# mfkiwl/HiSpMV

Measured on AMD Instinct MI355X. Metric: SpMV GFLOP/s, SuiteSparse set (20 matrices), fp32 y=alpha*A*x+beta*y, flops=2*(nnz+rows), higher is better.
Workload: dtype f32

## Files before the change

hispmv_amd/_lib.py:

```python
from __future__ import annotations

import ctypes as C
import os
from pathlib import Path

_HERE = Path(__file__).resolve().parent
LIB_PATH = Path(os.environ.get("HISPMV_LIB", _HERE / "lib" / "libhispmv.so"))

HISPMV_OK = 0
HISPMV_FULL = -1
HISPMV_EINVAL = -2
HISPMV_EDEVICE = -3
HISPMV_ESTATE = -4
HISPMV_ENOTDENSE = -5
HISPMV_EIO = -6
HISPMV_ENOMEM = -7


class MatrixInfo(C.Structure):
    _fields_ = [
        ("rows", C.c_int32), ("cols", C.c_int32), ("nnz", C.c_int64),
        ("is_dense", C.c_int32), ("loaded", C.c_int32),
        ("n_slices", C.c_int64), ("n_elems", C.c_int64), ("n_split_rows", C.c_int64),
        ("device_bytes", C.c_int64), ("prep_seconds", C.c_double),
        ("block_threads", C.c_int32), ("group_slices", C.c_int32), ("lds_bytes", C.c_int32), ("col_tiles", C.c_int32),
        ("carry_lookback", C.c_int32), ("col_tile_width", C.c_int32),
        ("col_tile_base", C.c_int32), ("compact_slices", C.c_int32),
        ("format", C.c_int32), ("tts_lines_per_gather", C.c_float), ("tile_kind", C.c_int32),
        ("batch_group_slices", C.c_int32),
    ]


_p = C.c_void_p
_i32p = C.POINTER(C.c_int32)
_i64p = C.POINTER(C.c_int64)
_u64p = C.POINTER(C.c_uint64)
_f32p = C.POINTER(C.c_float)

SIGNATURES = {
    "hispmv_prep_build_tts": (C.c_int, [_p, C.c_int64, C.c_int, C.POINTER(C.c_int64), C.POINTER(C.c_double)]),
    "hispmv_prep_tts_array": (C.c_void_p, [_p, C.c_int]),
    "hispmv_prep_tts_pieces": (C.c_int, [_p, C.POINTER(C.c_int64)]),
    "hispmv_version": (C.c_char_p, []),
    "hispmv_host_threads": (C.c_int, []),
    "hispmv_free_failures": (C.c_int64, []),
    "hispmv_boundary_pack": (C.c_int, [C.c_void_p, C.c_void_p, C.c_void_p, C.c_void_p, C.c_int32, C.c_void_p]),
    "hispmv_boundary_apply": (C.c_int, [C.c_void_p, C.c_void_p, C.c_void_p, C.c_void_p, C.c_int32, C.c_int32, C.c_void_p]),
    "hispmv_create": (C.c_int, [C.POINTER(_p), C.c_char_p] + [C.c_int] * 9),
    "hispmv_destroy": (None, [_p]),
    "hispmv_last_error": (C.c_char_p, [_p]),
    "hispmv_set_arena_bytes": (C.c_int, [_p, C.c_int64]),
    "hispmv_arena_bytes_used": (C.c_int64, [_p]),
    "hispmv_create_sparse_handle": (C.c_int, [_p, _p, _p, _p, C.c_int64, C.c_int32, C.c_int32]),
    "hispmv_create_sparse_handle_from_mtx": (C.c_int, [_p, C.c_char_p, C.c_int]),
    "hispmv_create_sparse_handle_from_csr": (C.c_int, [_p, _p, _p, _p, C.c_int32, C.c_int32]),
    "hispmv_create_dense_handle": (C.c_int, [_p, _p, C.c_int32, C.c_int32]),
    "hispmv_load_matrices": (C.c_int, [_p]),
    "hispmv_select_matrix": (C.c_int, [_p, C.c_uint32]),
    "hispmv_run_kernel": (C.c_int, [_p, _p, _p, _p, C.c_float, C.c_float]),
    "hispmv_linear": (C.c_int, [_p, C.c_int, _p, C.c_int64, _p, _p]),
    "hispmv_spmv_device": (C.c_int, [_p, C.c_int, _p, _p, _p, C.c_float, C.c_float, _p]),
    "hispmv_synchronize": (C.c_int, [_p]),
    "hispmv_last_kernel_ms": (C.c_float, [_p]),
    "hispmv_batch_graph_stats": (C.c_int, [_p, C.POINTER(C.c_int64)]),
    "hispmv_batch_call_info": (C.c_int, [_p, C.POINTER(C.c_int64)]),
    "hispmv_spmv_device_batch": (C.c_int, [_p, C.c_int32, _p, _p, _p, _p, C.c_float, C.c_float, _p]),
    "hispmv_set_value_updates": (C.c_int, [_p, C.c_int]),
    "hispmv_update_values": (C.c_int, [_p, C.c_int, _p, C.c_int64]),
    "hispmv_update_values_device": (C.c_int, [_p, C.c_int, _p, C.c_int64, _p]),
    "hispmv_value_update_info": (C.c_int, [_p, C.c_int, _i64p]),
    "hispmv_time_device": (C.c_float, [_p, C.c_int, _p, _p, _p, C.c_float, C.c_float, C.c_int]),
    "hispmv_get_matrix_info": (C.c_int, [_p, C.c_int, C.POINTER(MatrixInfo)]),
    "hispmv_num_matrices": (C.c_int, [_p]),
    "hispmv_prep_from_coo": (C.c_int, [C.POINTER(_p), _p, _p, _p, C.c_int64, C.c_int32, C.c_int32]),
    "hispmv_prep_from_coo_device": (C.c_int, [C.POINTER(_p), C.c_int, _p, _p, _p, C.c_int64, C.c_int32, C.c_int32, C.POINTER(C.c_double)]),
    "hispmv_prep_from_mtx": (C.c_int, [C.POINTER(_p), C.c_char_p, C.c_int]),
    "hispmv_prep_free": (None, [_p]),
    "hispmv_prep_last_error": (C.c_char_p, []),
    "hispmv_prep_dims": (C.c_int, [_p, _i64p]),
    "hispmv_prep_plan": (C.c_int, [_p, C.c_int, _i64p]),
    "hispmv_prep_choose_format": (C.c_int, [_p, C.c_int, _i64p]),
    "hispmv_prep_step_queue": (C.c_int, [_p, C.c_int32, _p, C.c_int32, C.c_int32, C.c_int32, _p, _p]),
    "hispmv_prep_window_membership": (C.c_int, [_p, C.c_int, C.c_void_p]),
    "hispmv_prep_apply_plan": (C.c_int, [_p, C.c_int, _i64p]),
    "hispmv_prep_groups": (_i32p, [_p]),
    "hispmv_prep_device_stream": (C.c_int, [_p, _i64p]),
    "hispmv_prep_device_array": (C.c_void_p, [_p, C.c_int]),
    "hispmv_prep_device_stream_on_device": (C.c_int, [_p, C.c_int, C.c_void_p, C.c_void_p]),
    "hispmv_prep_frags": (_i32p, [_p]),
    "hispmv_prep_value_layouts": (C.c_int, [C.POINTER(_p), _p, _p, _p, C.c_int64, C.c_int32, C.c_int32, C.c_int, _i64p]),
    "hispmv_prep_value_array": (C.c_void_p, [_p, C.c_int]),
    "hispmv_prep_csr_row_ptr": (_i64p, [_p]),
    "hispmv_prep_csr_col": (_i32p, [_p]),
    "hispmv_prep_csr_val": (_f32p, [_p]),
    "hispmv_prep_words": (_u64p, [_p]),
    "hispmv_prep_slice_hdr": (_i32p, [_p]),
    "hispmv_prep_fix": (_i32p, [_p]),
}


def _bind_single_hip_runtime() -> None:
    import importlib.util
    spec = importlib.util.find_spec("torch")
    if spec is None or not spec.origin:
        return
    cand = Path(spec.origin).parent / "lib" / "libamdhip64.so"
    if cand.exists():
        C.CDLL(str(cand), mode=C.RTLD_GLOBAL)


def _load() -> C.CDLL:
    if not LIB_PATH.exists():
        raise ImportError(
            f"{LIB_PATH} not found: the HIP library is not built. Run "
            "`python -c 'import __graft_entry__ as g; g.build()'` (or `make -C hispmv_amd/csrc`). "
            "There is no CPU fallback."
        )
    _bind_single_hip_runtime()
    lib = C.CDLL(str(LIB_PATH))
    for name, (res, args) in SIGNATURES.items():
        fn = getattr(lib, name)
        fn.restype = res
        fn.argtypes = args
    return lib


lib = _load()
```

hispmv_amd/csrc/hispmv_abi.cpp:

```cpp
#include "hispmv_ctx.h"

using namespace hispmv;

namespace {

thread_local std::string g_create_err;
thread_local std::string g_prep_err;

}

namespace hispmv {
int fail(hispmv_ctx* c, int code, const std::string& msg) {
    if (c) c->err = msg; else g_create_err = msg;
    return code;
}
int hip_fail(hispmv_ctx* c, hipError_t e, const char* what) {
    return fail(c, HISPMV_EDEVICE, std::string(what) + ": " + hipGetErrorString(e));
}
std::string& prep_error() { return g_prep_err; }
std::atomic<int64_t> g_free_failures{0};
int check_device_error(hispmv_ctx* c) {
    const int flag = *(volatile int*)c->h_err;
    if (flag) {
        *(volatile int*)c->h_err = 0;
// ... 437 lines not shown
            const int rc = check_updatable(c, nnz);
            if (rc != HISPMV_OK) return rc;
        }
        csr.col.assign(ci, ci + nnz);
        if (c->value_updates) { real.assign(va, va + nnz); const std::vector<float> pl = index_payloads(nnz); csr.val.assign(pl.begin(), pl.end()); }
        else csr.val.assign(va, va + nnz);
        for (int64_t k = 0; k < nnz; ++k) if (ci[k] < 0 || ci[k] >= cols) return fail(c, HISPMV_EINVAL, "CSR column outside matrix");
        sort_rows_by_column(csr);
        double t = std::chrono::duration<double>(std::chrono::steady_clock::now() - t0).count();
        return add_sparse(c, std::move(csr), t, nullptr, c->value_updates ? &real : nullptr);
    } catch (const std::bad_alloc&) { return fail(c, HISPMV_ENOMEM, "host out of memory");
    } catch (const std::exception& ex) { return fail(c, HISPMV_EINVAL, ex.what()); }
}

HISPMV_API int hispmv_create_dense_handle(hispmv_ctx* c, const float* vals, int32_t rows, int32_t cols) {
    if (!c) return HISPMV_EINVAL;
    std::lock_guard<std::mutex> g(c->mu);
    if (!c->dense_overlay)
        return fail(c, HISPMV_ENOTDENSE, "Hardware is not built with Dense Overlay, cannot support dense workload");
    if (rows <= 0 || cols <= 0 || !vals) return fail(c, HISPMV_EINVAL, "bad dense matrix arguments");
    try {
        auto t0 = std::chrono::steady_clock::now();
        auto m = std::make_unique<Matrix>();
        m->dense = true; m->rows = rows; m->cols = cols; m->nnz = (int64_t)rows * cols;
        m->device_bytes = m->nnz * 4;
        if (c->arena_used + m->device_bytes > c->arena_budget) return HISPMV_FULL;
        m->dense_host.assign(vals, vals + m->nnz);
        if (c->value_updates) { m->updatable = true; m->upd_n = m->nnz; m->upd_written = m->nnz; }
        m->prep_seconds = std::chrono::duration<double>(std::chrono::steady_clock::now() - t0).count();
        c->arena_used += m->device_bytes;
        m->index = (int)c->mats.size();
    c->mats.push_back(std::move(m));
        return (int)c->mats.size() - 1;
    } catch (const std::bad_alloc&) { return fail(c, HISPMV_ENOMEM, "host out of memory"); }
}

HISPMV_API int hispmv_load_matrices(hispmv_ctx* c) {
    if (!c) return HISPMV_EINVAL;
    std::lock_guard<std::mutex> g(c->mu);
    HIP_TRY(c, hipSetDevice(c->device));
    for (auto& mp : c->mats) {
        Matrix& m = *mp;
        if (m.loaded) continue;
        int rc;
        struct Scratch { std::vector<void*> v; void push_back(void* p) { v.push_back(p); } ~Scratch() { for (void* p : v) (void)hipFree(p); } } layout_scratch;
        std::vector<std::vector<int32_t>> tts_fix_rows;
        std::vector<std::vector<ValueChunk>> value_regions;
        std::vector<std::pair<int64_t, int64_t>> layout_bytes;
        if (m.updatable && !m.dense)
            for (const Matrix::Part& p : m.parts) {
                value_regions.push_back(value_chunks(p));
                layout_bytes.emplace_back(p.is_tts ? (int64_t)p.tts.words.size() : p.dstream.n_bytes, p.has_batch_layout ? p.batch_dstream.n_bytes : 0);
            }
        if (m.dense) {
            const float* d = nullptr;
            if ((rc = upload(c, m, m.dense_host.data(), m.dense_host.size(), &d)) != HISPMV_OK) return rc;
            m.d_dense = const_cast<float*>(d);
        } else if (m.format == 1) {
          for (Matrix::Part& p : m.parts) {
            TtsStream& ts = p.tts;
            tts_fix_rows.emplace_back();
            for (size_t k = 0; k + 3 < ts.fix.size(); k += 4) tts_fix_rows.back().push_back(ts.fix[k]);
            const uint8_t* dw = nullptr; const int32_t* dcb = nullptr; const uint16_t* dfl = nullptr; const int32_t* dci = nullptr;
            const TtsTile* dt = nullptr; const TtsBlock* db = nullptr;
            if ((rc = upload(c, m, ts.words.data(), ts.words.size(), &dw)) != HISPMV_OK) return rc;
            if ((rc = upload(c, m, ts.col_base.data(), ts.col_base.size(), &dcb)) != HISPMV_OK) return rc;
            if ((rc = upload(c, m, ts.flags.data(), ts.flags.size(), &dfl)) != HISPMV_OK) return rc;
            const uint16_t* dfh = nullptr;
            std::vector<uint32_t> planes;
            if (!ts.flags_hi.empty()) {
                planes.resize(ts.flags.size());
                for (size_t q = 0; q < planes.size(); ++q) planes[q] = (uint32_t)ts.flags[q] | ((uint32_t)ts.flags_hi[q] << 16);
                const uint32_t* dp = nullptr;
                if ((rc = upload(c, m, planes.data(), planes.size(), &dp)) != HISPMV_OK) return rc;
                HIP_TRY(c, hipStreamSynchronize(c->stream));
                dfh = (const uint16_t*)dp;
            }
            if ((rc = upload(c, m, ts.chunk_info.data(), ts.chunk_info.size(), &dci)) != HISPMV_OK) return rc;
            if ((rc = upload(c, m, ts.tiles.data(), ts.tiles.size(), &dt)) != HISPMV_OK) return rc;
            if ((rc = upload(c, m, ts.blocks.data(), ts.blocks.size(), &db)) != HISPMV_OK) return rc;
            TtsDeviceMatrix& d = p.tdev;
            d.words = dw; d.col_base = dcb; d.flags = dfl; d.flags_hi = dfh; d.chunk_info = (const int2*)dci; d.tiles = (const int4*)dt; d.blocks = (const int4*)db;
            d.n_tiles = (int32_t)ts.tiles.size(); d.rows = m.rows; d.cols = m.cols;
            if (!ts.fix.empty()) {
                const int32_t* dfix = nullptr;
                if ((rc = upload(c, m, ts.fix.data(), ts.fix.size(), &dfix)) != HISPMV_OK) return rc;
                void* carry = nullptr;
                HIP_TRY(c, hipMalloc(&carry, (size_t)std::max(ts.n_carry, 1) * kTtsMaxVectors * sizeof(float)));
                m.allocs.push_back(carry);
                HIP_TRY(c, hipMemsetAsync(carry, 0, (size_t)std::max(ts.n_carry, 1) * kTtsMaxVectors * sizeof(float), c->stream));
                d.n_carry = ts.n_carry;
                d.fix = (const int4*)dfix; d.n_fix = (int32_t)(ts.fix.size() / 4); d.carry = (float*)carry;
                p.dev.fix_short = d.fix; p.dev.n_fix_short = d.n_fix; p.dev.carry = d.carry; p.dev.n_fix_long = 0;
            }
            d.acc_floats = (ts.max_rows + 63) & ~63; d.threads = ts.geometry.threads;
            d.zero_fill = ts.geometry.zero_fill ? 1 : ts.geometry.gap_rows ? 2 : 0;
            d.staging_floats = ts.geometry.max_slots + 64;
            d.batch_stage_floats = ((ts.max_slots + kTtsChunk - 1) / kTtsChunk) * kTtsChunk + 64;
            d.xlds_floats = (m.cols <= kTtsXldsMax && std::getenv("HISPMV_TTS_XLDS")) ? ((m.cols + 63) & ~63) : 0;
            if (((size_t)d.acc_floats + (size_t)d.staging_floats + 64) * 4 > 160 * 1024 - 256) return fail(c, HISPMV_EINVAL, "internal: tile stream exceeds the LDS of a CU");
            HIP_TRY(c, hipStreamSynchronize(c->stream));
            p.tts = TtsStream{};
          }
        } else {
            for (auto& p : m.parts) {
                const uint8_t* dw = nullptr; const SliceHdr* dh = nullptr; const FixEntry *fs = nullptr, *fl = nullptr;
                const int32_t* dg = nullptr; const Frag* dfr = nullptr;
                const int64_t ns = p.st.n_slices;
                if ((rc = upload(c, m, p.dstream.groups.data(), p.dstream.groups.size(), &dg)) != HISPMV_OK) return rc;
                if ((rc = upload(c, m, p.plan.frags.data(), p.plan.frags.size(), &dfr)) != HISPMV_OK) return rc;
                const bool lay_out = p.dstream.bytes.empty() && p.dstream.n_bytes > 0;
                uint64_t* d_host_words = nullptr;
                if (!lay_out) {
                    if ((rc = upload(c, m, p.dstream.bytes.data(), p.dstream.bytes.size(), &dw)) != HISPMV_OK) return rc;
                } else {
                    if ((int64_t)p.st.words.size() != ns * kSliceElems) return fail(c, HISPMV_EINVAL, "internal: host words missing for the device layout");
                    void* blk = nullptr;
                    HIP_TRY(c, hipMalloc(&blk, (size_t)p.dstream.n_bytes));
                    m.allocs.push_back(blk);
                    dw = (const uint8_t*)blk;
                    HIP_TRY(c, hipMalloc((void**)&d_host_words, p.st.words.size() * sizeof(uint64_t)));
                    layout_scratch.push_back(d_host_words);
                    HIP_TRY(c, hipMemcpyAsync(d_host_words, p.st.words.data(), p.st.words.size() * sizeof(uint64_t), hipMemcpyHostToDevice, c->stream));
                }
                std::vector<SliceHdr>& hh = p.st.hdr;
                int max_rows = 1;
                for (int64_t sl = 0; sl < ns; ++sl) {
                    const int nr = (sl + 1 < ns ? hh[sl + 1].row_base : m.rows) - hh[sl].row_base;
                    hh[sl].x_base = nr;
                    hh[sl].x_span = (!p.plan.slice_spills.empty() && p.plan.slice_spills[(size_t)sl]) ? 1 : 0;
                    max_rows = std::max(max_rows, nr);
                }
                uint32_t* d_stray_cols = nullptr;
                if (!p.dstream.any_stray) {
                    if ((rc = upload(c, m, hh.data(), hh.size(), &dh)) != HISPMV_OK) return rc;
                } else if (lay_out) {
                    void* blk = nullptr;
                    const size_t hb = hh.size() * sizeof(SliceHdr), sb = (size_t)ns * kStraySlots * sizeof(uint32_t);
                    HIP_TRY(c, hipMalloc(&blk, hb + sb));
                    m.allocs.push_back(blk);
                    HIP_TRY(c, hipMemcpyAsync(blk, hh.data(), hb, hipMemcpyHostToDevice, c->stream));
                    HIP_TRY(c, hipMemsetAsync((char*)blk + hb, 0xff, sb, c->stream));
                    dh = (const SliceHdr*)blk;
                    d_stray_cols = (uint32_t*)((char*)blk + hb);
                } else {
                    void* blk = nullptr;
                    const size_t hb = hh.size() * sizeof(SliceHdr), sb = p.dstream.stray_cols.size() * sizeof(uint32_t);
                    HIP_TRY(c, hipMalloc(&blk, hb + sb));
                    m.allocs.push_back(blk);
                    HIP_TRY(c, hipMemcpyAsync(blk, hh.data(), hb, hipMemcpyHostToDevice, c->stream));
                    HIP_TRY(c, hipMemcpyAsync((char*)blk + hb, p.dstream.stray_cols.data(), sb, hipMemcpyHostToDevice, c->stream));
                    dh = (const SliceHdr*)blk;
                }
                if (lay_out) {
                    const int e = layout_on_device(d_host_words, ns, p.plan.group_slices, dg, p.plan.lds_floats, p.plan.block_threads / 64,
                                                   (uint8_t*)dw, d_stray_cols, c->stream);
                    if (e != 0) return hip_fail(c, (hipError_t)e, "layout_on_device");
                }
                if ((rc = upload(c, m, p.fix_short.data(), p.fix_short.size(), &fs)) != HISPMV_OK) return rc;
                if ((rc = upload(c, m, p.fix_long.data(), p.fix_long.size(), &fl)) != HISPMV_OK) return rc;
                void *carry = nullptr, *gran = nullptr, *ticket = nullptr;
                const size_t n1 = (size_t)std::max<int64_t>(ns, 1);
                HIP_TRY(c, hipMalloc(&carry, n1 * kMaxBatch * sizeof(float)));
                m.allocs.push_back(carry);
                HIP_TRY(c, hipMemsetAsync(carry, 0, n1 * kMaxBatch * sizeof(float), c->stream));
                HIP_TRY(c, hipMalloc(&gran, n1 * sizeof(unsigned long long)));
                m.allocs.push_back(gran);
                HIP_TRY(c, hipMemsetAsync(gran, 0, n1 * sizeof(unsigned long long), c->stream));
                HIP_TRY(c, hipMalloc(&ticket, sizeof(unsigned long long)));
                m.allocs.push_back(ticket);
                HIP_TRY(c, hipMemsetAsync(ticket, 0, sizeof(unsigned long long), c->stream));
                SpmvDeviceMatrix& d = p.dev;
                d.words = dw; d.hdr = (const int4*)dh; d.groups = (const int4*)dg; d.frags = (const int4*)dfr;
                d.fix_short = (const int4*)fs; d.fix_long = (const int4*)fl;
                d.carry = (float*)carry; d.gran = (unsigned long long*)gran; d.ticket = (unsigned long long*)ticket;
                d.err = c->d_err; d.launches = 0; d.ticket_launches = 0;
                d.n_slices = ns; d.n_groups = (ns + p.plan.group_slices - 1) / p.plan.group_slices;
                d.group_slices = p.plan.group_slices; d.block_threads = p.plan.block_threads;
                d.lds_floats = p.plan.lds_floats + p.dstream.stray_floats;
                d.ytile_floats = std::min(kSliceElems, (max_rows + 63) & ~63);
                const size_t lds_plain = (size_t)(d.lds_floats + d.ytile_floats * (d.block_threads / 64)) * 4;
                if (lds_plain > 160 * 1024 - 256) return fail(c, HISPMV_EINVAL, "internal: launch plan exceeds the LDS of a CU");
                const bool mailbox_fits = lds_plain + (size_t)d.group_slices * 8 <= 160 * 1024 - 256;
                d.n_fix_short = (int32_t)p.fix_short.size(); d.n_fix_long = (int32_t)p.fix_long.size();
                d.rows = m.rows; d.cols = m.cols;
                const int lds_b = std::max(1, (int)lds_plain + 64);
                const int per_cu = std::max(1, std::min({4, (160 * 1024) / lds_b, 16 / (d.block_threads / 64)}));
                const bool resident = d.n_groups <= (int64_t)c->n_cus * per_cu;
                const bool one_round = d.group_slices <= d.block_threads / 64;
                d.lookback = (c->carry_mode == 1 || c->carry_mode == 3 || (c->carry_mode == 2 && resident && one_round) ||
                              (c->carry_mode == 5 && resident)) && mailbox_fits;
                d.use_ticket = c->carry_mode == 3;
                if (m.parts.size() > 1) { d.lookback = false; d.use_ticket = false; }
                d.has_strays = p.dstream.stray_floats > 0;
                if (d.has_strays) { d.lookback = false; d.use_ticket = false; }
                if (p.has_batch_layout) {
                    SpmvDeviceMatrix b = d;
                    const int32_t* bg = nullptr; const Frag* bf = nullptr; const uint8_t* bw = nullptr; const SliceHdr* bh = nullptr;
                    if ((rc = upload(c, m, p.batch_dstream.groups.data(), p.batch_dstream.groups.size(), &bg)) != HISPMV_OK) return rc;
                    if ((rc = upload(c, m, p.batch_plan.frags.data(), p.batch_plan.frags.size(), &bf)) != HISPMV_OK) return rc;
                    std::vector<SliceHdr> bhh = hh;
                    for (int64_t sl = 0; sl < ns; ++sl) bhh[(size_t)sl].x_span = (!p.batch_plan.slice_spills.empty() && p.batch_plan.slice_spills[(size_t)sl]) ? 1 : 0;
                    uint32_t* b_stray = nullptr;
                    {
                        void* blk = nullptr;
                        const size_t hb = bhh.size() * sizeof(SliceHdr), sb = p.batch_dstream.any_stray ? (size_t)ns * kStraySlots * sizeof(uint32_t) : 0;
                        HIP_TRY(c, hipMalloc(&blk, hb + sb));
                        m.allocs.push_back(blk);
                        HIP_TRY(c, hipMemcpy(blk, bhh.data(), hb, hipMemcpyHostToDevice));
                        if (sb && !p.batch_dstream.stray_cols.empty()) HIP_TRY(c, hipMemcpy((char*)blk + hb, p.batch_dstream.stray_cols.data(), sb, hipMemcpyHostToDevice));
                        else if (sb) HIP_TRY(c, hipMemsetAsync((char*)blk + hb, 0xff, sb, c->stream));
                        bh = (const SliceHdr*)blk;
                        b_stray = sb ? (uint32_t*)((char*)blk + hb) : nullptr;
                    }
                    if (!p.batch_dstream.bytes.empty()) {
                        if ((rc = upload(c, m, p.batch_dstream.bytes.data(), p.batch_dstream.bytes.size(), &bw)) != HISPMV_OK) return rc;
                    } else {
                        void* blk = nullptr; uint64_t* tmp = nullptr;
                        HIP_TRY(c, hipMalloc(&blk, (size_t)p.batch_dstream.n_bytes));
                        m.allocs.push_back(blk);
                        bw = (const uint8_t*)blk;
                        HIP_TRY(c, hipMalloc((void**)&tmp, p.batch_words.size() * sizeof(uint64_t)));
                        layout_scratch.push_back(tmp);
                        HIP_TRY(c, hipMemcpyAsync(tmp, p.batch_words.data(), p.batch_words.size() * sizeof(uint64_t), hipMemcpyHostToDevice, c->stream));
                        const int e = layout_on_device(tmp, ns, p.batch_plan.group_slices, bg, p.batch_plan.lds_floats, p.batch_plan.block_threads / 64, (uint8_t*)blk, b_stray, c->stream);
                        if (e != 0) return hip_fail(c, (hipError_t)e, "layout_on_device");
                    }
                    b.words = bw; b.hdr = (const int4*)bh; b.groups = (const int4*)bg; b.frags = (const int4*)bf;
                    b.group_slices = p.batch_plan.group_slices; b.n_groups = (ns + p.batch_plan.group_slices - 1) / p.batch_plan.group_slices;
                    b.lds_floats = p.batch_plan.lds_floats + p.batch_dstream.stray_floats;
                    b.has_strays = p.batch_dstream.stray_floats > 0;
                    b.lookback = false; b.use_ticket = false;
                    if ((size_t)(b.lds_floats + b.ytile_floats * (b.block_threads / 64)) * 4 <= 160 * 1024 - 256) { p.batch_dev = b; p.has_batch_dev = true; }
                }
            }
        }
        if (!m.dense && m.parts.size() > 1) {
            void* yp = nullptr;
            HIP_TRY(c, hipMalloc(&yp, (m.parts.size() - 1) * (size_t)kMaxBatch * m.rows * sizeof(float)));
            m.allocs.push_back(yp);
            m.d_ypart = (float*)yp;
            bool fusable = m.parts.size() <= (size_t)kTailMaxParts;
            for (auto& p : m.parts) fusable = fusable && (p.is_tts || p.fix_long.empty());
            if (fusable) {
                std::vector<int32_t> of((size_t)m.parts.size() * m.rows, -1);
                for (size_t t = 0; t < m.parts.size(); ++t) {
                    int32_t* o = of.data() + t * (size_t)m.rows;
                    if (m.parts[t].is_tts) { const std::vector<int32_t>& f = tts_fix_rows[t]; for (size_t k = 0; k < f.size(); ++k) o[f[k]] = (int32_t)k; }
                    else for (size_t k = 0; k < m.parts[t].fix_short.size(); ++k) o[m.parts[t].fix_short[k].row] = (int32_t)k;
                }
                const int32_t* d_of = nullptr;
                if ((rc = upload(c, m, of.data(), of.size(), &d_of)) != HISPMV_OK) return rc;
                HIP_TRY(c, hipStreamSynchronize(c->stream));
                m.d_fix_of_row = const_cast<int32_t*>(d_of);
            }
        }
        if (m.updatable && !m.dense && (rc = load_value_map(c, m, value_regions, layout_bytes)) != HISPMV_OK) return rc;
        HIP_TRY(c, hipStreamSynchronize(c->stream));
        for (auto& p : m.parts) { p.st = SliceStream{}; p.fix_short = {}; p.fix_long = {}; p.plan.groups = {}; p.plan.frags = {}; p.dstream = DeviceStream{};
                                  p.batch_plan.groups = {}; p.batch_plan.frags = {}; p.batch_plan.slice_spills = {}; p.batch_dstream = DeviceStream{}; p.batch_words = WordVec(); }
        m.dense_host = {};
        m.loaded = true;
    }
    return HISPMV_OK;
}

HISPMV_API int hispmv_select_matrix(hispmv_ctx* c, uint32_t idx) {
    if (!c) return HISPMV_EINVAL;
    std::lock_guard<std::mutex> g(c->mu);
    if (idx >= c->mats.size()) return fail(c, HISPMV_EINVAL, "Matrix idx out of range");
    c->selected = (int)idx;
    return HISPMV_OK;
}

static int run_host_vectors(hispmv_ctx* c, Matrix& m, const float* x, int64_t num_vecs, const float* bias,
                            float* y, float alpha, float beta, bool is_linear) {
    HIP_TRY(c, hipSetDevice(c->device));
    int rc;
    const int64_t nx = (((int64_t)m.cols * num_vecs + 63) / 64) * 64, nb = m.rows, ny = (int64_t)m.rows * num_vecs;
    if ((rc = ensure_vec(c, &c->d_x, &c->cap_x, nx + nb)) != HISPMV_OK) return rc;
    if ((rc = ensure_vec(c, &c->d_y, &c->cap_y, ny)) != HISPMV_OK) return rc;
    float* const d_x = c->d_x;
// ... 195 lines not shown
```

hispmv_amd/csrc/hispmv_batch.cpp:

```cpp
#include "hispmv_ctx.h"

using namespace hispmv;

namespace hispmv {

void free_batch_plans(hispmv_ctx* c) {
    for (auto& p : c->batch_plans) {
        for (auto& g : p.slot) {
            if (g.launched && g.done) (void)hipEventSynchronize(g.done);
            if (g.exec) { (void)hipGraphExecDestroy(g.exec); g.exec = nullptr; }
            if (g.done) { (void)hipEventDestroy(g.done); g.done = nullptr; }
            g.launched = false;
        }
        if (p.graph_src) { (void)hipGraphDestroy(p.graph_src); p.graph_src = nullptr; }
        for (auto& l : p.launches) { dev_free(l.d_table); dev_free(l.d_table2); dev_free(l.d_items); dev_free(l.d_sync); }
    }
    c->batch_plans.clear();
}

}

static int build_batch_plan_with(hispmv_ctx* c, hispmv_ctx::BatchPlan& plan, int32_t n, const int32_t* idx, const float* const* d_x,
                                 const float* const* bias, float* const* d_y, float beta, bool long_groups, bool& used_long_groups, bool& step_taken);
static int build_batch_plan(hispmv_ctx* c, hispmv_ctx::BatchPlan& plan, int32_t n, const int32_t* idx, const float* const* d_x,
                            const float* const* bias, float* const* d_y, float beta) {
    bool used = false, step = false;
    int rc = build_batch_plan_with(c, plan, n, idx, d_x, bias, d_y, beta, true, used, step);
    if (rc == HISPMV_OK && used && !step) {
        for (auto& l : plan.launches) { dev_free(l.d_table); dev_free(l.d_table2); dev_free(l.d_items); dev_free(l.d_sync); }
        plan.launches.clear();
        rc = build_batch_plan_with(c, plan, n, idx, d_x, bias, d_y, beta, false, used, step);
    }
    return rc;
}
static int build_batch_plan_with(hispmv_ctx* c, hispmv_ctx::BatchPlan& plan, int32_t n, const int32_t* idx, const float* const* d_x,
                                 const float* const* bias, float* const* d_y, float beta, bool long_groups, bool& used_long_groups, bool& step_taken) {
    used_long_groups = false; step_taken = false;
    struct Ref { int i; size_t t; };
    struct Item { std::vector<Ref> refs; int threads; int64_t slices; bool strays = false; };
    std::vector<Item> items;
    std::vector<Ref> refs;
    const bool shared_chip = c->batch_streams > 1 && plan.stream_bytes >= c->batch_streams_min_bytes && !std::getenv("HISPMV_NO_BATCH_LAYOUT");
    auto dev_of = [&](const Ref& r) -> SpmvDeviceMatrix& {
        Matrix::Part& p = c->mats[idx[r.i]]->parts[r.t];
        if (shared_chip && long_groups && p.has_batch_dev) { used_long_groups = true; return p.batch_dev; }
        return p.dev;
    };
    auto out_of = [&](const Ref& r) -> float* {
        Matrix& m = *c->mats[idx[r.i]];
        return r.t == 0 ? d_y[r.i] : m.d_ypart + (r.t - 1) * (size_t)kMaxBatch * m.rows;
    };
    const bool pin = !std::getenv("HISPMV_NO_XCD_PIN");
    auto upload_table0 = [&](hispmv_ctx::BatchLaunch& l, const void* host, size_t bytes) -> int {
        HIP_TRY(c, hipMalloc(&l.d_table, bytes));
        HIP_TRY(c, hipMemcpy(l.d_table, host, bytes, hipMemcpyHostToDevice));
        return HISPMV_OK;
    };
    {
        std::vector<int> dense;
        for (int i = 0; i < n; ++i) if (c->mats[idx[i]]->dense) dense.push_back(i);
        std::stable_sort(dense.begin(), dense.end(), [&](int a, int b) {
            const Matrix& ma = *c->mats[idx[a]]; const Matrix& mb = *c->mats[idx[b]];
            return (int64_t)ma.rows * ma.cols > (int64_t)mb.rows * mb.cols;
        });
        for (size_t k0 = 0; k0 < dense.size(); k0 += kMultiMax) {
            hispmv_ctx::BatchLaunch l;
            l.kind = 4;
            for (size_t k = k0; k < std::min(dense.size(), k0 + (size_t)kMultiMax); ++k) {
                const int i = dense[k];
                const Matrix& m = *c->mats[idx[i]];
                l.gemv.push_back(GemvEntry{m.d_dense, d_x[i], bias[i], d_y[i], m.rows, m.cols, beta, 0});
            }
            plan.launches.push_back(std::move(l));
            const int rc0 = upload_table0(plan.launches.back(), plan.launches.back().gemv.data(), plan.launches.back().gemv.size() * sizeof(GemvEntry));
            if (rc0 != HISPMV_OK) return rc0;
        }
    }
    auto tts_class = [](const Matrix& m) {
        return m.parts[0].tdev.staging_floats + (m.parts.size() == 1 && tts_x_in_lds(m.parts[0].tdev, 1) ? (1 << 24) : 0) + (m.parts[0].tdev.zero_fill << 25);
    };
    std::vector<int> tts_classes;
    for (int i = 0; i < n; ++i) {
        const Matrix& m = *c->mats[idx[i]];
        if (m.dense || m.format != 1) continue;
        const int cls = tts_class(m);
        if (std::find(tts_classes.begin(), tts_classes.end(), cls) == tts_classes.end()) tts_classes.push_back(cls);
    }
    std::sort(tts_classes.begin(), tts_classes.end());
    for (const int geometry : tts_classes) {
        hispmv_ctx::BatchLaunch l;
        l.kind = 3;
        auto flush = [&]() -> int {
            if (l.tts.empty()) return HISPMV_OK;
            plan.launches.push_back(std::move(l));
            const int rc0 = upload_table0(plan.launches.back(), plan.launches.back().tts.data(), plan.launches.back().tts.size() * sizeof(TtsEntry));
            l = hispmv_ctx::BatchLaunch{};
            l.kind = 3;
            return rc0;
        };
        std::vector<int> order;
// ... 28 lines not shown
            for (size_t t = 0; t < m.parts.size(); ++t) { it.refs.push_back(Ref{i, t}); it.slices += m.parts[t].dev.n_slices; }
            items.push_back(std::move(it));
        } else {
            for (size_t t = 0; t < m.parts.size(); ++t) { const SpmvDeviceMatrix& d = dev_of(Ref{i, t}); items.push_back(Item{{Ref{i, t}}, d.block_threads, d.n_slices, d.has_strays}); }
        }
    }
    std::stable_sort(items.begin(), items.end(), [&](const Item& a, const Item& b) {
        if (a.threads != b.threads) return a.threads > b.threads;
        if (a.strays != b.strays) return !a.strays;
        return a.slices > b.slices;
    });
    const size_t first_slice_launch = plan.launches.size();
    for (const Item& it : items) for (const Ref& r : it.refs) refs.push_back(r);
    auto upload_table = [&](hispmv_ctx::BatchLaunch& l, const void* host, size_t bytes) -> int {
        HIP_TRY(c, hipMalloc(&l.d_table, bytes));
        HIP_TRY(c, hipMemcpy(l.d_table, host, bytes, hipMemcpyHostToDevice));
        return HISPMV_OK;
    };
    int rc;
    for (size_t k = 0; k < items.size();) {
        const int threads = items[k].threads;
        hispmv_ctx::BatchLaunch l;
        l.kind = 0;
        std::vector<MultiEntry> entries;
        const bool strays = items[k].strays;
        while (k < items.size() && items[k].threads == threads && items[k].strays == strays && entries.size() + items[k].refs.size() <= (size_t)kMultiMax) {
            for (const Ref& r : items[k].refs) {
                SpmvDeviceMatrix& d = dev_of(r);
                MultiEntry e{};
                e.words = d.words; e.hdr = d.hdr; e.groups = d.groups; e.frags = d.frags;
                e.x = d_x[r.i]; e.bias = r.t == 0 ? bias[r.i] : nullptr; e.y = out_of(r); e.carry = d.carry;
                e.n_slices = d.n_slices; e.group_slices = d.group_slices; e.lds_floats = d.lds_floats; e.ytile_floats = d.ytile_floats;
                e.cols = d.cols; e.rows = d.rows;
                e.beta = r.t == 0 ? beta : 0.0f;
                entries.push_back(e);
                l.parts.push_back(&d);
            }
            l.item_tiles.push_back((uint8_t)items[k].refs.size());
            ++k;
        }
        l.multi = entries;
        plan.launches.push_back(std::move(l));
        if ((rc = upload_table(plan.launches.back(), entries.data(), entries.size() * sizeof(MultiEntry))) != HISPMV_OK) return rc;
    }
    if (c->batch_order == 1) {
        std::vector<hispmv_ctx::BatchLaunch> slices(std::make_move_iterator(plan.launches.begin() + (long)first_slice_launch),
                                                    std::make_move_iterator(plan.launches.end()));
        plan.launches.erase(plan.launches.begin() + (long)first_slice_launch, plan.launches.end());
        std::reverse(slices.begin(), slices.end());
        std::vector<hispmv_ctx::BatchLaunch> rest = std::move(plan.launches);
        plan.launches.clear();
        for (auto& l : slices) plan.launches.push_back(std::move(l));
        for (auto& l : rest) plan.launches.push_back(std::move(l));
    }
    if (c->step_kernel && shared_chip && !c->cu_split && !c->batch_graphs) {
        bool ok = true;
        size_t lds = 0;
        bool strays = false;
        for (const auto& l : plan.launches) {
            if (l.kind == 4) ok = false;
            if (l.kind == 0) {
                for (uint8_t t : l.item_tiles) ok = ok && t == 1;
                for (const SpmvDeviceMatrix* d : l.parts) {
                    ok = ok && (d->block_threads == 1024 || d->block_threads == 256);
                    const size_t one = ((size_t)d->lds_floats + (size_t)d->ytile_floats * (d->block_threads / 64)) * sizeof(float);
                    lds = std::max(lds, d->block_threads == 256 ? 4 * one : one);
                    strays = strays || d->has_strays;
                }
            }
            if (l.kind == 3) {
                for (uint8_t t : l.item_tiles) ok = ok && t == 1;
                for (const TtsEntry& e : l.tts) {
                    ok = ok && e.m.zero_fill == 0 && e.m.threads == 1024 && !tts_x_in_lds(e.m, 1);
                    lds = std::max(lds, tts_tile_lds_bytes(e.m));
                }
            }
        }
        ok = ok && lds <= 160 * 1024 - 256;
        if (ok) {
            struct QItem { uint32_t a, b; double cost; int cls; };
            std::vector<QItem> q[2];
            std::vector<MultiEntry> slice_table;
            std::vector<TtsEntry> tts_table;
            for (const auto& l : plan.launches) {
                if (l.kind == 0) {
                    for (size_t e = 0; e < l.multi.size(); ++e) {
                        const SpmvDeviceMatrix& d = *l.parts[e];
                        const uint32_t entry = (uint32_t)slice_table.size();
                        slice_table.push_back(l.multi[e]);
                        const int64_t ng = d.n_slices > 0 ? d.n_groups : 0;
                        const bool window = d.lds_floats > 0;
                        const double per_slice = window ? 0.27 : 0.68;
                        if (d.block_threads == 1024) {
                            for (int64_t g = 0; g < ng; ++g) {
                                const int64_t n_here = std::min<int64_t>(d.group_slices, d.n_slices - g * d.group_slices);
                                q[0].push_back(QItem{0u | (entry << 8), (uint32_t)g, 1.0 + per_slice * (double)n_here + (double)d.lds_floats * 4.0 / 40000.0, 0});
                            }
                        } else {
                            for (int64_t g = 0; g < ng; g += 4) {
                                const int64_t n_here = std::min<int64_t>(d.group_slices, d.n_slices - g * d.group_slices);
                                static const double f256 = std::getenv("HISPMV_STEP_COST256") ? std::atof(std::getenv("HISPMV_STEP_COST256")) : 8.0;
                                q[0].push_back(QItem{1u | (entry << 8), (uint32_t)g, 1.0 + f256 * (double)n_here + (double)d.lds_floats * 4.0 / 40000.0, 0});
                            }
                        }
                    }
                }
                if (l.kind == 3) {
                    for (const TtsEntry& te : l.tts) {
                        const uint32_t entry = (uint32_t)tts_table.size();
                        tts_table.push_back(te);
                        std::vector<int4> tiles((size_t)te.m.n_tiles);
                        HIP_TRY(c, hipMemcpy(tiles.data(), te.m.tiles, tiles.size() * sizeof(int4), hipMemcpyDeviceToHost));
                        int n_blocks = 0;
                        for (const int4& t : tiles) n_blocks = std::max(n_blocks, t.z + t.w);
                        std::vector<int4> blocks((size_t)n_blocks * 2);
                        if (n_blocks > 0) HIP_TRY(c, hipMemcpy(blocks.data(), te.m.blocks, blocks.size() * sizeof(int4), hipMemcpyDeviceToHost));
                        double lines = 23.0;
                        for (int i = 0; i < n; ++i) { const Matrix& m = *c->mats[idx[i]]; if (!m.dense && m.format == 1 && m.parts[0].tdev.words == te.m.words && m.tts_lines_per_gather > 0) lines = m.tts_lines_per_gather; }
                        static const double tile_scale = std::getenv("HISPMV_STEP_TILE_SCALE") ? std::atof(std::getenv("HISPMV_STEP_TILE_SCALE")) : 1.0;
                        const double per_slice = tile_scale * 0.85 * (50.0 + 2.8 * lines) / (50.0 + 2.8 * 23.0);
                        for (int t = 0; t < te.m.n_tiles; ++t) {
                            int64_t sl = 0;
                            for (int b = tiles[(size_t)t].z; b < tiles[(size_t)t].z + tiles[(size_t)t].w; ++b) sl += blocks[(size_t)b * 2].y;
                            q[1].push_back(QItem{2u | (entry << 8), (uint32_t)t, 2.0 + per_slice * (double)sl + 0.5 * (double)tiles[(size_t)t].w, 1});
                        }
                    }
                }
            }
            if (slice_table.size() < (1u << 20) && tts_table.size() < (1u << 20) && !q[0].empty()) {
                const int W = std::max(1, c->n_cus);
                std::vector<double> cost[2];
                for (int k = 0; k < 2; ++k) for (const QItem& it : q[k]) cost[k].push_back(it.cost);
                std::vector<QItem> order;
                for (const auto& pr : order_step_queue(cost[0], cost[1], W, c->step_order)) order.push_back(q[pr.first][(size_t)pr.second]);
                std::vector<uint32_t> packed;
                packed.reserve(order.size() * 2);
                for (const QItem& it : order) { packed.push_back(it.a); packed.push_back(it.b); }
                hispmv_ctx::BatchLaunch L;
                L.kind = 6;
                L.n_items = (unsigned)order.size();
                L.step_workgroups = (int)std::min<size_t>((size_t)W, order.size());
                L.step_lds = lds;
                L.step_strays = strays;
                for (const auto& l : plan.launches) L.weight += l.weight;
                std::vector<hispmv_ctx::BatchLaunch> keep;
                for (auto& l : plan.launches) {
                    if (l.kind == 0 || l.kind == 3) { dev_free(l.d_table); dev_free(l.d_table2); }
                    else keep.push_back(std::move(l));
                }
                plan.launches.clear();
                plan.launches.push_back(std::move(L));
                for (auto& l : keep) plan.launches.push_back(std::move(l));
                hispmv_ctx::BatchLaunch& S = plan.launches.front();
                if (!slice_table.empty()) {
                    HIP_TRY(c, hipMalloc(&S.d_table, slice_table.size() * sizeof(MultiEntry)));
                    HIP_TRY(c, hipMemcpy(S.d_table, slice_table.data(), slice_table.size() * sizeof(MultiEntry), hipMemcpyHostToDevice));
                }
                if (!tts_table.empty()) {
                    HIP_TRY(c, hipMalloc(&S.d_table2, tts_table.size() * sizeof(TtsEntry)));
                    HIP_TRY(c, hipMemcpy(S.d_table2, tts_table.data(), tts_table.size() * sizeof(TtsEntry), hipMemcpyHostToDevice));
                }
                HIP_TRY(c, hipMalloc(&S.d_items, packed.size() * sizeof(uint32_t)));
                HIP_TRY(c, hipMemcpy(S.d_items, packed.data(), packed.size() * sizeof(uint32_t), hipMemcpyHostToDevice));
                HIP_TRY(c, hipMalloc((void**)&S.d_sync, 2 * sizeof(unsigned)));
                HIP_TRY(c, hipMemset(S.d_sync, 0, 2 * sizeof(unsigned)));
                step_taken = true;
            }
        }
    }
    if (long_groups && used_long_groups && !step_taken) return HISPMV_OK;
    std::vector<Ref> fixrefs = refs;
    for (int i = 0; i < n; ++i) {
        const Matrix& m = *c->mats[idx[i]];
        if (!m.dense && m.format == 1)
            for (size_t t = 0; t < m.parts.size(); ++t) if (m.parts[t].tdev.n_fix > 0) fixrefs.push_back(Ref{i, t});
    }
    {
        plan.lanes = plan.stream_bytes >= c->batch_streams_min_bytes ? c->batch_streams : 1;
        std::vector<hispmv_ctx::BatchLaunch*> mains;
        for (auto& l : plan.launches) {
            if (l.kind == 0) for (const SpmvDeviceMatrix* d : l.parts) l.weight += d->n_slices * (int64_t)kWideSliceBytes;
            if (l.kind == 4) for (const GemvEntry& e : l.gemv) l.weight += 4 * (int64_t)e.rows * e.cols;
            mains.push_back(&l);
        }
        plan.lanes = std::max(1, std::min<int>(plan.lanes, (int)mains.size()));
        int k = 0;
        for (hispmv_ctx::BatchLaunch* l : mains) l->lane = k++ % plan.lanes;
        if (c->batch_lanes_heavy_first && plan.lanes >= 2) {
            std::vector<int64_t> load((size_t)plan.lanes, 0);
            for (hispmv_ctx::BatchLaunch* l : mains) load[(size_t)l->lane] += l->weight;
            const int heavy = (int)(std::max_element(load.begin(), load.end()) - load.begin());
            for (hispmv_ctx::BatchLaunch* l : mains) l->lane = l->lane == heavy ? 0 : l->lane == 0 ? heavy : l->lane;
            std::stable_sort(plan.launches.begin(), plan.launches.end(), [](const hispmv_ctx::BatchLaunch& x, const hispmv_ctx::BatchLaunch& y) { return x.lane < y.lane; });
        }
    }
    std::vector<int> tiled;
    bool fused = !std::getenv("HISPMV_NO_FUSED_TAIL");
    for (int i = 0; i < n; ++i) {
        const Matrix& m = *c->mats[idx[i]];
        if (m.dense || m.parts.size() < 2) continue;
        tiled.push_back(i);
        fused = fused && m.d_fix_of_row != nullptr;
    }
    if (fused) {
        std::vector<Ref> plain;
        for (const Ref& r : fixrefs) if (c->mats[idx[r.i]]->parts.size() < 2) plain.push_back(r);
        fused = plain.size() <= (size_t)kMultiMax && tiled.size() <= (size_t)kMultiMax;
        static const bool lane_tails = std::getenv("HISPMV_LANE_TAILS") != nullptr;
        if (fused && lane_tails && plan.lanes > 1) {
            auto lane_of_out = [&](const float* out, const SpmvDeviceMatrix* dev) -> int {
                for (const auto& l : plan.launches) {
                    if (l.kind == 0) for (const SpmvDeviceMatrix* d : l.parts) if (d == dev) return l.lane;
                    if (l.kind == 3) for (const TtsEntry& e : l.tts) if (e.y == out) return l.lane;
                }
                return -1;
            };
            std::vector<std::vector<Ref>> lane_plain((size_t)plan.lanes);
            std::vector<std::vector<int>> lane_tiled((size_t)plan.lanes);
            std::vector<Ref> rest_plain; std::vector<int> rest_tiled;
            for (const Ref& r : plain) { const int ln = lane_of_out(out_of(r), &dev_of(r)); if (ln >= 0) lane_plain[(size_t)ln].push_back(r); else rest_plain.push_back(r); }
            for (int i : tiled) {
                Matrix& m = *c->mats[idx[i]];
                int ln = -2;
                for (size_t t = 0; t < m.parts.size(); ++t) { const int q = lane_of_out(out_of(Ref{i, t}), &m.parts[t].dev); ln = ln == -2 ? q : (ln == q ? ln : -1); }
                if (ln >= 0) lane_tiled[(size_t)ln].push_back(i); else rest_tiled.push_back(i);
            }
            auto make_tail = [&](const std::vector<Ref>& pl, const std::vector<int>& ti, int lane, bool in_lane) -> int {
                hispmv_ctx::BatchLaunch l;
                l.kind = 5; l.lane = lane; l.in_lane = in_lane;
                std::vector<MultiFixEntry> fix; std::vector<TailMergeEntry> mrg;
                bool any = !ti.empty();
                for (const Ref& r : pl) {
                    SpmvDeviceMatrix& d = dev_of(r);
                    fix.push_back(MultiFixEntry{d.fix_short, d.carry, out_of(r), d.n_fix_short, 0});
                    l.fix_counts.push_back(d.n_fix_short);
                    l.parts.push_back(&d); l.ys.push_back(out_of(r));
                    any = any || d.n_fix_short > 0 || d.n_fix_long > 0;
                }
                for (int i : ti) {
                    Matrix& m = *c->mats[idx[i]];
                    TailMergeEntry e{};
                    e.y = d_y[i]; e.parts = m.d_ypart; e.part_stride = (long long)kMaxBatch * m.rows; e.n_parts = (int32_t)m.parts.size() - 1; e.rows = m.rows;
                    e.fix_of_row = m.d_fix_of_row;
                    for (size_t t = 0; t < m.parts.size(); ++t) { e.fix[t] = m.parts[t].dev.fix_short; e.carry[t] = m.parts[t].dev.carry; }
                    mrg.push_back(e);
                    l.rows.push_back(m.rows);
                }
                if (!any) return HISPMV_OK;
                plan.launches.push_back(std::move(l));
// ... 255 lines not shown
```

hispmv_amd/csrc/hispmv_ctx.h:

```cpp
#pragma once
#include "../../include/hispmv.h"

#include <hip/hip_runtime_api.h>

#include <algorithm>
#include <atomic>
#include <chrono>
#include <cstdio>
#include <cstdlib>
#include <cstring>
#include <memory>
#include <mutex>
#include <stdexcept>
#include <string>
#include <vector>

#include "hispmv_choose.h"
#include "hispmv_kernels.h"
#include "hispmv_plan.h"
#include "hispmv_prep.h"
#include "hispmv_prep_device.h"
#include "hispmv_tts.h"
#include "hispmv_update.h"

#define HISPMV_API extern "C" __attribute__((visibility("default")))


namespace hispmv {

struct Matrix {
    bool dense = false;
    int32_t rows = 0, cols = 0;
    int64_t nnz = 0;
    double prep_seconds = 0;
    int64_t device_bytes = 0;
    bool loaded = false;
    struct Part : HostPart {
        TtsDeviceMatrix tdev;
        hispmv::SpmvDeviceMatrix dev;
        hispmv::SpmvDeviceMatrix batch_dev;
        bool has_batch_dev = false;
    };
    std::vector<Part> parts;
    std::vector<float> dense_host;
    int64_t n_slices = 0, n_elems = 0, n_split = 0, compact_slices = 0;
    int plan_threads = 0, plan_group = 0, plan_lds = 0, col_tile_width = 0, col_tile_base = 0;
    int tile_kind = 0;
    int format = 0;
    int index = -1;
    double tts_lines_per_gather = 0;
    bool l2_tiles = false;
    float* d_dense = nullptr;
    float* d_ypart = nullptr;
    int32_t* d_fix_of_row = nullptr;
    bool updatable = false;
    int64_t upd_n = 0;
    int64_t map_slots = 0;
    int64_t upd_written = 0;
    std::vector<float> upd_values;
    int32_t* d_map = nullptr;
    ValueChunkDev* d_upd_table = nullptr;
    std::vector<void*> allocs;
};

}

struct hispmv_ctx {
    int device = 0;
    int num_ch_A = 0, num_ch_B = 0, num_ch_C = 0, urams_per_pe = 0, fp_acc_latency = 0;
    bool dense_overlay = false, pre_accumulator = false, row_dist_net = false;
    hipStream_t stream = nullptr;
    hipStream_t user_stream = nullptr;
    hipStream_t side[2] = {nullptr, nullptr};
    bool cu_split = false;
    hipEvent_t ev_fork = nullptr, ev_join[2] = {nullptr, nullptr};
    int batch_streams = 2;
    int batch_order = 0;
    bool batch_lanes_heavy_first = true;
    bool step_kernel = true;
    int step_order = 0;
    bool batch_graphs = false;
    int64_t batch_streams_min_bytes = 256ll << 20;
    hipEvent_t ev0 = nullptr, ev1 = nullptr;
    float last_ms = -1.0f;
    std::mutex mu;
    std::string err;
    std::vector<std::unique_ptr<hispmv::Matrix>> mats;
    int selected = -1;
    int64_t arena_budget = 0, arena_used = 0;
    float *d_x = nullptr, *d_y = nullptr;
    int64_t cap_x = 0, cap_y = 0;
    int* h_err = nullptr;
    int* d_err = nullptr;
    float* h_stage = nullptr;
    float* d_stage = nullptr;
    int64_t cap_stage = 0;
    bool value_updates = false;
    float* h_upd = nullptr;
    int64_t cap_h_upd = 0;
    float* d_upd = nullptr;
    int64_t cap_d_upd = 0;
    struct BatchLaunch {
        int kind = 0;
        std::vector<hispmv::TtsEntry> tts;
        std::vector<hispmv::GemvEntry> gemv;
        std::vector<const hispmv::SpmvDeviceMatrix*> parts;
        std::vector<float*> ys;
        std::vector<int32_t> rows;
        std::vector<uint8_t> item_tiles;
        std::vector<int32_t> fix_counts;
        std::vector<hispmv::MultiEntry> multi;
        void* d_table = nullptr;
        void* d_table2 = nullptr;
        void* d_items = nullptr;
        unsigned* d_sync = nullptr;
        unsigned n_items = 0;
        int step_workgroups = 0;
        size_t step_lds = 0;
        bool step_strays = false;
        int lane = 0;
        bool in_lane = false;
        int64_t weight = 0;
    };
    struct BatchPlan {
        std::vector<uint64_t> key;
        std::vector<BatchLaunch> launches;
        int64_t stream_bytes = 0;
        int lanes = 1;
        struct GraphSlot {
            hipGraphExec_t exec = nullptr;
            float alpha = 0.0f;
            hipEvent_t done = nullptr;
            bool launched = false;
            uint64_t last_use = 0;
        } slot[2];
        uint64_t use_counter = 0;
        hipGraph_t graph_src = nullptr;
        int runs = 0;
    };
    std::vector<BatchPlan> batch_plans;
    int64_t graph_instantiations = 0, graph_alpha_updates = 0;
    int64_t last_batch[4] = {-1, 0, 0, 0};
    int carry_mode = 2;
    int prep_mode = 2;
    hispmv::DevicePrepTimes last_prep_times;
    hispmv::FormatOptions format_opts;
    int n_cus = 256;
};

struct hispmv_prep {
    hispmv::Csr csr;
    hispmv::SliceStream st;
    hispmv::LaunchPlan plan;
    hispmv::TtsStream tts;
    hispmv::DeviceStream dstream;
    std::vector<uint8_t> vl_real, vl_index;
    std::vector<int32_t> vl_map;
    std::vector<int64_t> vl_chunks;
};


namespace hispmv {

int fail(hispmv_ctx* c, int code, const std::string& msg);
int hip_fail(hispmv_ctx* c, hipError_t e, const char* what);
std::string& prep_error();
#define HIP_TRY(c, call)                                                 \
    do {                                                                 \
        hipError_t e_ = (call);                                          \
        if (e_ != hipSuccess) return ::hispmv::hip_fail((c), e_, #call); \
    } while (0)

extern std::atomic<int64_t> g_free_failures;
template <class T> void dev_free(T*& p) {
    if (p && hipFree((void*)p) != hipSuccess) { g_free_failures++; (void)hipGetLastError(); }
    p = nullptr;
}
template <class T> void host_free(T*& p) {
    if (p && hipHostFree((void*)p) != hipSuccess) { g_free_failures++; (void)hipGetLastError(); }
    p = nullptr;
}

int check_device_error(hispmv_ctx* c);
void free_batch_plans(hispmv_ctx* c);
int spmv_batch_locked(hispmv_ctx* c, int32_t n, const int32_t* idx, const float* const* d_x, const float* const* d_bias,
                      float* const* d_y, float alpha, float beta, hipStream_t s);

}
```

hispmv_amd/csrc/hispmv_kernels.h:

```cpp
#pragma once
#include <hip/hip_runtime_api.h>
#include <hip/hip_vector_types.h>
#include <cstdint>

namespace hispmv {

struct SpmvDeviceMatrix {
    const void* words = nullptr;
    const int4* hdr = nullptr;
    const int4* fix_short = nullptr;
    const int4* fix_long = nullptr;
    const int4* groups = nullptr;
    const int4* frags = nullptr;
    float* carry = nullptr;
    int64_t n_groups = 0;
    int32_t group_slices = 8;
    int32_t block_threads = 256;
    int32_t lds_floats = 0;
    bool has_strays = false;
    int32_t ytile_floats = 1024;
    bool lookback = true;
    unsigned long long* gran = nullptr;
    unsigned long long* ticket = nullptr;
    int* err = nullptr;
// ... 20 lines not shown
    int32_t n_tiles = 0, rows = 0, cols = 0;
    int32_t n_carry = 0;
    int32_t acc_floats = 0, staging_floats = 0;
    int32_t xlds_floats = 0;
    int32_t batch_stage_floats = 0;
    int32_t threads = 512;
};
struct TtsEntry {
    TtsDeviceMatrix m;
    const float* x; const float* bias; float* y;
    float beta; int32_t pad;
};

struct GemvEntry {
    const float* W; const float* x; const float* bias; float* y;
    int32_t rows, cols;
    float beta; int32_t pad;
};

struct LookbackArgs {
    unsigned long long* gran;
    unsigned long long* ticket;
    int* err;
    unsigned long long ticket_base;
    unsigned epoch;
    int use_ticket;
};

struct MultiEntry {
    const void* words; const int4* hdr; const int4* groups; const int4* frags;
    const float* x; const float* bias; float* y; float* carry;
    long long n_slices;
    int32_t group_slices, lds_floats, ytile_floats, cols, rows;
    float beta;
};
struct MultiFixEntry { const int4* fix; const float* carry; float* y; int32_t n, pad; };
struct MultiMergeEntry { float* y; const float* parts; long long part_stride; int32_t n_parts, rows; };
constexpr int kTailMaxParts = 9;
struct TailMergeEntry {
    float* y; const float* parts; long long part_stride; int32_t n_parts, rows;
    const int32_t* fix_of_row;
    const int4* fix[kTailMaxParts];
    const float* carry[kTailMaxParts];
};
constexpr int kMultiMax = 32;
struct MultiPrefix {
    int32_t n, pad;
    long long begin[kMultiMax + 1];
    uint8_t first[kMultiMax];
    uint8_t tiles[kMultiMax];
};

constexpr int kMaxBatch = 4;

hipError_t prepare_spmv_kernels();

hipError_t launch_spmv(SpmvDeviceMatrix& m, const float* x, const float* bias, float* y,
                       float alpha, float beta, hipStream_t stream, bool fixup_only = false);

int spmv_batch_width(const SpmvDeviceMatrix& m, int64_t vecs);
hipError_t launch_spmv_batched(SpmvDeviceMatrix& m, int nv, const float* x, const float* bias, int bias_stride, float* y,
                               float alpha, float beta, hipStream_t stream);

hipError_t launch_spmv_multi(const SpmvDeviceMatrix* const* parts, int n, const uint8_t* item_tiles, int n_items,
                             const MultiEntry* d_table, float alpha, hipStream_t stream);
hipError_t launch_merge_parts(float* y, const float* parts, int n_parts, int64_t part_stride, int32_t rows, int nv,
                              int64_t y_stride, int64_t vec_stride, hipStream_t stream);
hipError_t launch_merge_multi(const int32_t* rows, int n, const MultiMergeEntry* d_table, hipStream_t stream);
hipError_t launch_fixup_multi(const SpmvDeviceMatrix* const* parts, float* const* ys, int n, const MultiFixEntry* d_fix_table,
                              float alpha, hipStream_t stream);
hipError_t launch_fixup_long(const SpmvDeviceMatrix& m, float* y, float alpha, hipStream_t stream);
hipError_t launch_tail_multi(const int32_t* fix_counts, int n_fix, const MultiFixEntry* d_fix_table, const int32_t* merge_rows, int n_merge,
                             const TailMergeEntry* d_merge_table, float alpha, hipStream_t stream);

hipError_t launch_tts(const TtsDeviceMatrix& m, const float* x, const float* bias, float* y, float alpha, float beta, hipStream_t stream);
constexpr int kTtsMaxVectors = 8;
constexpr int kTtsXldsMax = 16 * 1024;
bool tts_x_in_lds(const TtsDeviceMatrix& m, int nv);
int tts_batch_width(const TtsDeviceMatrix& m, int64_t vecs);
hipError_t launch_tts_batched(const TtsDeviceMatrix& m, int nv, const float* x, const float* bias, float* y, float alpha, float beta, hipStream_t stream);
hipError_t launch_tts_multi(const TtsEntry* entries, int n, const uint8_t* item_parts, int n_items, const TtsEntry* d_table, float alpha,
                            hipStream_t stream);

struct StepArgs { const MultiEntry* slice_table; const TtsEntry* tts_table; const int2* items; unsigned* sync; unsigned n_items; float alpha; int pad, ticket_word; };
hipError_t launch_spmv_step(const MultiEntry* d_slice_table, const TtsEntry* d_tts_table, const void* d_items, unsigned n_items,
                            unsigned* d_sync, int workgroups, size_t lds_bytes, bool strays, float alpha, hipStream_t stream);
size_t tts_tile_lds_bytes(const TtsDeviceMatrix& m);

hipError_t launch_gemv(const float* W, int32_t rows, int32_t cols, const float* x, const float* bias,
                       float* y, float alpha, float beta, hipStream_t stream);
hipError_t launch_gemv_multi(const GemvEntry* entries, int n, const GemvEntry* d_table, float alpha, hipStream_t stream);
hipError_t launch_gemv_batched(const float* W, int32_t rows, int32_t cols, int64_t vecs, const float* x, const float* bias,
                               float* y, float alpha, float beta, hipStream_t stream);

hipError_t graph_set_alpha(hipGraphExec_t exec, hipGraph_t graph, float alpha);

hipError_t launch_fetch_vectors(const float* src, float* dst, int64_t n_floats, hipStream_t stream);
hipError_t launch_boundary_pack(const float* const* last, const float* mask, float* send, int n, hipStream_t stream);
hipError_t launch_boundary_apply(float* const* first, const float* recv, const float* weights, int n, int world,
                                 hipStream_t stream);

}
```

hispmv_amd/csrc/hispmv_kernels.hip:

```cpp
#include <hip/hip_runtime.h>

#include "hispmv_format.h"
#include "hispmv_kernels.h"
#include <algorithm>
#include <cstdlib>
#include <vector>

#ifndef HISPMV_TTS_EXPERIMENT
#define HISPMV_TTS_EXPERIMENT 0
#endif

namespace hispmv {

#ifdef HISPMV_WG_TRACE
__device__ unsigned long long* g_wgt_buf = nullptr;
__device__ unsigned g_wgt_cap = 0;
struct WgTrace {
    unsigned long long t0;
    __device__ __forceinline__ void begin() { t0 = __builtin_amdgcn_s_memrealtime(); }
    __device__ __forceinline__ void end(int kind, int entry, long long item) {
        __syncthreads();
        if (threadIdx.x == 0 && g_wgt_buf) {
            const unsigned long long t1 = __builtin_amdgcn_s_memrealtime();
            unsigned hw, xcc;
// ... 34 lines not shown
}
template <int CTRL, int ROWMASK>
__device__ __forceinline__ void seg_scan_step(float& v, unsigned long long F) {
    const float vp = i2f(__builtin_amdgcn_update_dpp(0, f2i(v), CTRL, ROWMASK, 0xf, false));
    v = __builtin_amdgcn_inverse_ballot_w64(F) ? v : v + vp;
}
__device__ __forceinline__ void seg_scan_wave(float& v, const ScanFlags& s) {
    seg_scan_step<0x111, 0xf>(v, s.f[0]);
    seg_scan_step<0x112, 0xf>(v, s.f[1]);
    seg_scan_step<0x114, 0xf>(v, s.f[2]);
    seg_scan_step<0x118, 0xf>(v, s.f[3]);
    seg_scan_step<0x142, 0xa>(v, s.f[4]);
    seg_scan_step<0x143, 0xc>(v, s.f[5]);
}

__device__ __forceinline__ float wave_sum(float v) {
    v += i2f(__builtin_amdgcn_update_dpp(0, f2i(v), 0x111, 0xf, 0xf, false));
    v += i2f(__builtin_amdgcn_update_dpp(0, f2i(v), 0x112, 0xf, 0xf, false));
    v += i2f(__builtin_amdgcn_update_dpp(0, f2i(v), 0x114, 0xf, 0xf, false));
    v += i2f(__builtin_amdgcn_update_dpp(0, f2i(v), 0x118, 0xf, 0xf, false));
    v += i2f(__builtin_amdgcn_update_dpp(0, f2i(v), 0x142, 0xa, 0xf, false));
    v += i2f(__builtin_amdgcn_update_dpp(0, f2i(v), 0x143, 0xc, 0xf, false));
    return i2f(__builtin_amdgcn_readlane(f2i(v), 63));
}

constexpr int kTtsChunkSlots = 1024;
constexpr int kLookbackSpinMax = 1 << 22;

__device__ __forceinline__ int lanes_below(unsigned long long mask) {
    return __builtin_amdgcn_mbcnt_hi((unsigned)(mask >> 32), __builtin_amdgcn_mbcnt_lo((unsigned)mask, 0));
}

typedef __attribute__((address_space(3))) unsigned long long lds_u64;
__device__ __forceinline__ void mbox_store(lds_u64* p, unsigned long long v) {
    __hip_atomic_store(p, v, __ATOMIC_RELAXED, __HIP_MEMORY_SCOPE_WORKGROUP);
}
__device__ __forceinline__ unsigned long long mbox_load(lds_u64* p) {
    return __hip_atomic_load(p, __ATOMIC_RELAXED, __HIP_MEMORY_SCOPE_WORKGROUP);
}

__device__ __forceinline__ float lookback_chain(const LookbackArgs& lb, lds_u64* local,
                                                long long first, long long cur, int chain_len, int lane) {
    float part = 0.0f;
    for (int k = lane; k < chain_len; k += 64) {
        const long long src = cur - chain_len + k;
        unsigned long long v;
        int spins = 0;
        if (src >= first) {
            v = mbox_load(local + (src - first));
            while ((unsigned)(v >> 32) != lb.epoch && spins < kLookbackSpinMax) {
                __builtin_amdgcn_s_sleep(1);
                v = mbox_load(local + (src - first));
                ++spins;
            }
        } else {
            const unsigned long long* g = lb.gran + src;
            v = __hip_atomic_load(g, __ATOMIC_RELAXED, __HIP_MEMORY_SCOPE_AGENT);
            while ((unsigned)(v >> 32) != lb.epoch && spins < kLookbackSpinMax) {
                __builtin_amdgcn_s_sleep(2);
                v = __hip_atomic_load(g, __ATOMIC_RELAXED, __HIP_MEMORY_SCOPE_AGENT);
                ++spins;
            }
        }
        if ((unsigned)(v >> 32) != lb.epoch) *lb.err = 1;
        part += i2f((int)(unsigned)v);
    }
    return wave_sum(part);
}

#define HISPMV_GLOBAL __attribute__((address_space(1)))
__device__ __forceinline__ uint4 load_words(const uint4* p) {
    typedef unsigned int u4v __attribute__((ext_vector_type(4)));
    const u4v v = __builtin_nontemporal_load((const HISPMV_GLOBAL u4v*)p);
    return uint4{v.x, v.y, v.z, v.w};
}
__device__ __forceinline__ uint2 load_words2(const uint2* p) {
    typedef unsigned int u2v __attribute__((ext_vector_type(2)));
    const u2v v = __builtin_nontemporal_load((const HISPMV_GLOBAL u2v*)p);
    return uint2{v.x, v.y};
}
__device__ __forceinline__ int4 load_int4(const int4* p) {
    typedef int i4v __attribute__((ext_vector_type(4)));
    const i4v v = *(const HISPMV_GLOBAL i4v*)p;
    return int4{v.x, v.y, v.z, v.w};
}
__device__ __forceinline__ float4 load_float4(const float4* p) {
    typedef float f4v __attribute__((ext_vector_type(4)));
    const f4v v = *(const HISPMV_GLOBAL f4v*)p;
    return float4{v.x, v.y, v.z, v.w};
}
__device__ __forceinline__ void store_float(float* p, float v) { *(HISPMV_GLOBAL float*)p = v; }
__device__ __forceinline__ int2 load_int2(const int2* p) {
    typedef int i2v __attribute__((ext_vector_type(2)));
    const i2v v = *(const HISPMV_GLOBAL i2v*)p;
    return int2{v.x, v.y};
}

template <bool COMPACT> struct SliceRaw;
template <> struct SliceRaw<true>  { uint4 v[kSliceSteps]; uint2 m[kSliceSteps]; };
template <> struct SliceRaw<false> { uint4 v[kSliceSteps]; uint4 m[kSliceSteps]; };
template <bool COMPACT>
__device__ __forceinline__ void request_slice(SliceRaw<COMPACT>& s, const char* base, int lane) {
    const uint4* pv = (const uint4*)base + lane;
#pragma unroll
    for (int j = 0; j < kSliceSteps; ++j) s.v[j] = load_words(pv + j * 64);
    if constexpr (COMPACT) {
        const uint2* pm = (const uint2*)(base + kSliceElems * 4) + lane;
#pragma unroll
        for (int j = 0; j < kSliceSteps; ++j) s.m[j] = load_words2(pm + j * 64);
    } else {
        const uint4* pm = (const uint4*)(base + kSliceElems * 4) + lane;
#pragma unroll
        for (int j = 0; j < kSliceSteps; ++j) s.m[j] = load_words(pm + j * 64);
    }
}
template <bool COMPACT>
__device__ __forceinline__ void decode_metas(const SliceRaw<COMPACT>& s, unsigned (&c)[kSliceSteps * kLaneElems]) {
    if constexpr (COMPACT) {
#pragma unroll
        for (int j = 0; j < kSliceSteps; ++j) {
            const unsigned a = s.m[j].x, b = s.m[j].y;
            c[4 * j + 0] = ((a & 0x8000u) << 16) | (a & 0x7fffu);
            c[4 * j + 1] = (a & 0x80000000u) | ((a >> 16) & 0x7fffu);
            c[4 * j + 2] = ((b & 0x8000u) << 16) | (b & 0x7fffu);
            c[4 * j + 3] = (b & 0x80000000u) | ((b >> 16) & 0x7fffu);
        }
    } else {
#pragma unroll
        for (int j = 0; j < kSliceSteps; ++j) { c[4 * j + 0] = s.m[j].x; c[4 * j + 1] = s.m[j].y; c[4 * j + 2] = s.m[j].z; c[4 * j + 3] = s.m[j].w; }
    }
}

__device__ __forceinline__ void scan_step(const float (&p)[kLaneElems], bool e0, bool e1, bool e2, bool e3, float& carry_step,
                                          float (&t)[kLaneElems]) {
    const float s0 = p[0];
    const float s1 = e0 ? p[1] : s0 + p[1];
    const float s2 = e1 ? p[2] : s1 + p[2];
    const float s3 = e2 ? p[3] : s2 + p[3];
    float v = e3 ? 0.0f : s3;
    const ScanFlags F = scan_flags(__builtin_amdgcn_ballot_w64(e0 | e1 | e2 | e3));
    seg_scan_wave(v, F);
    v = __builtin_amdgcn_inverse_ballot_w64(F.f[6]) ? v : v + carry_step;
    const float cin = i2f(__builtin_amdgcn_update_dpp(f2i(carry_step), f2i(v), 0x138, 0xf, 0xf, false));
    carry_step = i2f(__builtin_amdgcn_readlane(f2i(v), 63));
    t[0] = cin + s0;
    t[1] = e0 ? s1 : cin + s1;
    t[2] = (e0 | e1) ? s2 : cin + s2;
    t[3] = (e0 | e1 | e2) ? s3 : cin + s3;
}

__device__ __forceinline__ void stage_fragments(const int4* __restrict__ frags, int first, int count, const float* x, float* win,
                                                int cols, int lane, int wave, int n_waves) {
    constexpr int kU = 8;
    int4 fr = wave < count ? load_int4(frags + first + wave) : int4{0, 0, 0, 0};
    for (int f = wave; f < count; f += n_waves) {
        const int col0 = __builtin_amdgcn_readfirstlane(fr.x), n4 = __builtin_amdgcn_readfirstlane(fr.y) >> 2;
        const int off = __builtin_amdgcn_readfirstlane(fr.z);
        if (f + n_waves < count) fr = load_int4(frags + first + f + n_waves);
        const float4* src = (const float4*)(x + col0);
        float4* dst = (float4*)(win + off);
        const int inside = cols - col0 >= 4 * n4 ? n4 : (cols > col0 ? (cols - col0) >> 2 : 0);
        int i0 = 0;
        for (; inside - i0 > 128; i0 += 64 * kU) {
            float4 v[kU];
#pragma unroll
            for (int u = 0; u < kU; ++u) {
// ... 241 lines not shown
            float bb[4] = {0.0f, 0.0f, 0.0f, 0.0f};
            if (HAS_BETA) {
#pragma unroll
                for (int u = 0; u < 4; ++u) {
                    const int i = i0 + 64 * u + lane;
                    bb[u] = i2f((int)__builtin_amdgcn_raw_buffer_load_b32(rb, i < n_rows ? (unsigned)(row_first + i) << 2 : kNoAccess, 0, 0));
                }
            }
#pragma unroll
            for (int u = 0; u < 4; ++u) {
                const int i = i0 + 64 * u + lane;
                const float tt = i < n_rows ? ytile[i] : 0.0f;
                __builtin_amdgcn_raw_buffer_store_b32((unsigned)f2i(HAS_BETA ? alpha * tt + beta * bb[u] : alpha * tt), ry,
                                                      i < n_rows ? (unsigned)(row_first + i) << 2 : kNoAccess, 0, 0);
            }
        }
        for (int i = lane; LOOKBACK && i < n_rows; i += 64) {
            const float tt = ytile[i];
            const unsigned dst = (held && i == 0) ? kNoAccess : (unsigned)(row_first + i) << 2;
            if (HAS_BETA) {
                const float b = (i < 64) ? bpre0 : (i < 128) ? bpre1
                              : i2f((int)__builtin_amdgcn_raw_buffer_load_b32(rb, (unsigned)(row_first + i) << 2, 0, 0));
                if (LOOKBACK && deferred && i == 0) { def_t = tt; def_b = b; }
                if (LOOKBACK && rolling && i == 0) { pend_t = tt; pend_b = b; }
                __builtin_amdgcn_raw_buffer_store_b32((unsigned)f2i(alpha * tt + beta * b), ry, dst, 0, 0);
            } else {
                if (LOOKBACK && deferred && i == 0) def_t = tt;
                if (LOOKBACK && rolling && i == 0) pend_t = tt;
                __builtin_amdgcn_raw_buffer_store_b32((unsigned)f2i(alpha * tt), ry, dst, 0, 0);
            }
        }
    }
    if (!LOOKBACK) {
        __builtin_amdgcn_raw_buffer_store_b32((unsigned)f2i(HAS_BETA ? alpha * out_t0 + beta * out_b0 : alpha * out_t0), ry, out_d0, 0, 0);
        __builtin_amdgcn_raw_buffer_store_b32((unsigned)f2i(HAS_BETA ? alpha * out_t1 + beta * out_b1 : alpha * out_t1), ry, out_d1, 0, 0);
        __builtin_amdgcn_raw_buffer_store_b32((unsigned)f2i(out_carry), rc, out_dc, 0, 0);
    }
    if (LOOKBACK && pend_slice >= 0) {
        const float chain = lookback_chain(lb, mbox, first, pend_slice, pend_len, lane);
        if (lane == 0) {
            const float tt = pend_t + chain;
            __builtin_amdgcn_raw_buffer_store_b32((unsigned)f2i(HAS_BETA ? alpha * tt + beta * pend_b : alpha * tt), ry,
                                                  (unsigned)pend_row << 2, 0, 0);
        }
    }
    if (LOOKBACK && def_slice >= 0) {
        const float chain = lookback_chain(lb, mbox, first, def_slice, def_len, lane);
        if (lane == 0) {
            const float tt = def_t + chain;
            __builtin_amdgcn_raw_buffer_store_b32((unsigned)f2i(HAS_BETA ? alpha * tt + beta * def_b : alpha * tt), ry,
                                                  (unsigned)def_row << 2, 0, 0);
        }
    }
}

template <bool HAS_BETA, bool USE_LDS, bool LOOKBACK, bool STRAYS = false>
__device__ __forceinline__ void slices_body(
    const char* __restrict__ stream, const int4* __restrict__ hdr, const int4* __restrict__ groups,
    const int4* __restrict__ frags, const float* __restrict__ x, const float* bias, float* y,
    float* __restrict__ carry, float alpha, float beta, long long n_slices, int group_slices,
    int lds_floats, int ytile_floats, int cols, int rows, const LookbackArgs& lb, long long group, const SubBlock sb) {
    __shared__ long long s_group;
    if (LOOKBACK) {
        if (lb.use_ticket) {
            if (threadIdx.x == 0)
                s_group = (long long)(__hip_atomic_fetch_add(lb.ticket, 1ull, __ATOMIC_RELAXED, __HIP_MEMORY_SCOPE_AGENT) - lb.ticket_base);
            __syncthreads();
            group = s_group;
        }
    }
    if constexpr (USE_LDS) {
        const int4 g = group * group_slices < n_slices ? load_int4(groups + group) : int4{0, 0, 0, 0};
        if (__builtin_amdgcn_readfirstlane(g.w) != 0)
            slices_group<HAS_BETA, true, LOOKBACK, true, STRAYS>(stream, hdr, groups, frags, x, bias, y, carry, alpha, beta, n_slices, group_slices,
                                                         lds_floats, ytile_floats, cols, rows, lb, group, g, sb);
        else
            slices_group<HAS_BETA, true, LOOKBACK, false>(stream, hdr, groups, frags, x, bias, y, carry, alpha, beta, n_slices, group_slices,
                                                          lds_floats, ytile_floats, cols, rows, lb, group, g, sb);
    } else {
        slices_group<HAS_BETA, false, LOOKBACK, false>(stream, hdr, groups, frags, x, bias, y, carry, alpha, beta, n_slices, group_slices,
                                                       lds_floats, ytile_floats, cols, rows, lb, group, int4{0, 0, 0, 0}, sb);
    }
}
template <bool HAS_BETA, bool USE_LDS, bool LOOKBACK, bool STRAYS = false>
__device__ __forceinline__ void slices_body(
    const char* __restrict__ stream, const int4* __restrict__ hdr, const int4* __restrict__ groups,
    const int4* __restrict__ frags, const float* __restrict__ x, const float* bias, float* y,
    float* __restrict__ carry, float alpha, float beta, long long n_slices, int group_slices,
    int lds_floats, int ytile_floats, int cols, int rows, const LookbackArgs& lb, long long group) {
    slices_body<HAS_BETA, USE_LDS, LOOKBACK, STRAYS>(stream, hdr, groups, frags, x, bias, y, carry, alpha, beta, n_slices, group_slices,
                                                     lds_floats, ytile_floats, cols, rows, lb, group, SubBlock::whole());
}

template <bool HAS_BETA, bool USE_LDS, bool LOOKBACK, bool STRAYS = false>
__global__ __launch_bounds__(1024) void spmv_slices_kernel(
    const char* __restrict__ words, const int4* __restrict__ hdr, const int4* __restrict__ groups,
    const int4* __restrict__ frags, const float* __restrict__ x, const float* bias, float* y,
    float* __restrict__ carry, float alpha, float beta, long long n_slices, int group_slices,
    int lds_floats, int ytile_floats, int cols, int rows, LookbackArgs lb) {
    slices_body<HAS_BETA, USE_LDS, LOOKBACK, STRAYS>(words, hdr, groups, frags, x, bias, y, carry, alpha, beta, n_slices, group_slices,
                                             lds_floats, ytile_floats, cols, rows, lb, (long long)blockIdx.x);
}

template <bool STRAYS>
__global__ __launch_bounds__(1024) void spmv_slices_multi_kernel(const MultiEntry* __restrict__ table, MultiPrefix prefix, float alpha) {
    int k = 0;
#pragma unroll 1
    while (k + 1 < prefix.n && (long long)blockIdx.x >= prefix.begin[k + 1]) ++k;
    long long group = (long long)blockIdx.x - prefix.begin[k];
    int e = prefix.first[k];
    const int tiles = prefix.tiles[k];
    if (tiles > 1) {
        const int per = 8 / tiles, res = (int)(group & 7);
        e += res / per;
        group = (group >> 3) * per + (res % per);
    }
    const MultiEntry t = table[e];
    if (group * t.group_slices >= t.n_slices) return;
    WGT_BEGIN();
    const LookbackArgs lb{};
    if (t.beta != 0.0f)
        slices_body<true, true, false, STRAYS>((const char*)t.words, t.hdr, t.groups, t.frags, t.x, t.bias, t.y, t.carry, alpha, t.beta,
                                       t.n_slices, t.group_slices, t.lds_floats, t.ytile_floats, t.cols, t.rows, lb, group);
    else
        slices_body<false, true, false, STRAYS>((const char*)t.words, t.hdr, t.groups, t.frags, t.x, t.y, t.y, t.carry, alpha, 0.0f,
                                        t.n_slices, t.group_slices, t.lds_floats, t.ytile_floats, t.cols, t.rows, lb, group);
    WGT_END(blockDim.x == 1024 ? 1 : 2, e, group);
}

__global__ __launch_bounds__(256) void spmv_fixup_multi_kernel(const MultiFixEntry* __restrict__ table, MultiPrefix prefix, float alpha) {
    int e = 0;
#pragma unroll 1
    while (e + 1 < prefix.n && (long long)blockIdx.x >= prefix.begin[e + 1]) ++e;
    const MultiFixEntry t = table[e];
    const int i = (int)(blockIdx.x - prefix.begin[e]) * blockDim.x + threadIdx.x;
    if (i >= t.n) return;
    const int4 f = t.fix[i];
    float s = 0.0f;
    for (int k = 0; k < f.z; ++k) s += t.carry[f.y + k];
    t.y[f.x] += alpha * s;
}

__global__ __launch_bounds__(256) void spmv_merge_parts_kernel(float* __restrict__ y, const float* __restrict__ parts, int n_parts,
                                                               long long part_stride, int rows, long long y_stride, long long vec_stride) {
    const int i = blockIdx.x * blockDim.x + threadIdx.x;
    if (i >= rows) return;
    y += blockIdx.y * y_stride;
    parts += blockIdx.y * vec_stride;
    float s = y[i];
    for (int t = 0; t < n_parts; ++t) s += parts[(size_t)t * part_stride + i];
    y[i] = s;
}
__global__ __launch_bounds__(256) void spmv_merge_multi_kernel(const MultiMergeEntry* __restrict__ table, MultiPrefix prefix) {
    int e = 0;
#pragma unroll 1
    while (e + 1 < prefix.n && (long long)blockIdx.x >= prefix.begin[e + 1]) ++e;
    const MultiMergeEntry t = table[e];
    const int i = (int)(blockIdx.x - prefix.begin[e]) * blockDim.x + threadIdx.x;
    if (i >= t.rows) return;
    float s = t.y[i];
    for (int k = 0; k < t.n_parts; ++k) s += t.parts[(size_t)k * t.part_stride + i];
    t.y[i] = s;
}

__global__ __launch_bounds__(256) void spmv_tail_multi_kernel(const MultiFixEntry* __restrict__ fix_table, MultiPrefix fix_prefix,
                                                              const TailMergeEntry* __restrict__ merge_table, MultiPrefix merge_prefix, float alpha) {
// ... 409 lines not shown
        raised = true;
    }
    bool strays = false;
    for (int i = 0; i < n; ++i) strays = strays || parts[i]->has_strays;
    if (g > 0 && strays) hipLaunchKernelGGL(spmv_slices_multi_kernel<true>, dim3((unsigned)g), dim3(threads), lds, stream, d_table, px, alpha);
    else if (g > 0) hipLaunchKernelGGL(spmv_slices_multi_kernel<false>, dim3((unsigned)g), dim3(threads), lds, stream, d_table, px, alpha);
    return hipGetLastError();
}

hipError_t launch_merge_parts(float* y, const float* parts, int n_parts, int64_t part_stride, int32_t rows, int nv,
                              int64_t y_stride, int64_t vec_stride, hipStream_t stream) {
    (void)hipGetLastError();
    if (n_parts <= 0 || rows <= 0) return hipSuccess;
    hipLaunchKernelGGL(spmv_merge_parts_kernel, dim3((unsigned)((rows + 255) / 256), (unsigned)nv), dim3(256), 0, stream,
                       y, parts, n_parts, (long long)part_stride, rows, (long long)y_stride, (long long)vec_stride);
    return hipGetLastError();
}

hipError_t launch_merge_multi(const int32_t* rows, int n, const MultiMergeEntry* d_table, hipStream_t stream) {
    (void)hipGetLastError();
    if (n <= 0) return hipSuccess;
    if (n > kMultiMax) return hipErrorInvalidValue;
    MultiPrefix px{};
    px.n = n;
    long long b = 0;
    for (int i = 0; i < n; ++i) { px.begin[i] = b; b += (rows[i] + 255) / 256; }
    px.begin[n] = b;
    if (b > 0) hipLaunchKernelGGL(spmv_merge_multi_kernel, dim3((unsigned)b), dim3(256), 0, stream, d_table, px);
    return hipGetLastError();
}

hipError_t launch_fixup_long(const SpmvDeviceMatrix& m, float* y, float alpha, hipStream_t stream) {
    (void)hipGetLastError();
    if (m.n_fix_long > 0)
        hipLaunchKernelGGL(spmv_fixup_long_kernel, dim3((m.n_fix_long + 3) / 4), dim3(256), 0, stream, m.fix_long, m.n_fix_long, m.carry, y, alpha, 0LL, 0LL);
    return hipGetLastError();
}

hipError_t launch_tail_multi(const int32_t* fix_counts, int n_fix, const MultiFixEntry* d_fix_table, const int32_t* merge_rows, int n_merge,
                             const TailMergeEntry* d_merge_table, float alpha, hipStream_t stream) {
    (void)hipGetLastError();
    if (n_fix > kMultiMax || n_merge > kMultiMax) return hipErrorInvalidValue;
    MultiPrefix fx{}, mx{};
    fx.n = n_fix; mx.n = n_merge;
    long long fb = 0, mb = 0;
    for (int i = 0; i < n_fix; ++i) { fx.begin[i] = fb; fb += (fix_counts[i] + 255) / 256; }
    fx.begin[n_fix] = fb;
    for (int i = 0; i < n_merge; ++i) { mx.begin[i] = mb; mb += (merge_rows[i] + 255) / 256; }
    mx.begin[n_merge] = mb;
    if (fb + mb > 0x7fffffffLL) return hipErrorInvalidValue;
    if (fb + mb > 0) hipLaunchKernelGGL(spmv_tail_multi_kernel, dim3((unsigned)(fb + mb)), dim3(256), 0, stream, d_fix_table, fx, d_merge_table, mx, alpha);
    return hipGetLastError();
}

hipError_t launch_fixup_multi(const SpmvDeviceMatrix* const* parts, float* const* ys, int n, const MultiFixEntry* d_fix_table,
                              float alpha, hipStream_t stream) {
    (void)hipGetLastError();
    if (n <= 0) return hipSuccess;
    if (n > kMultiMax) return hipErrorInvalidValue;
    MultiPrefix fx{};
    fx.n = n;
    long long fb = 0;
    for (int i = 0; i < n; ++i) { fx.begin[i] = fb; fb += (parts[i]->n_fix_short + 255) / 256; }
    fx.begin[n] = fb;
    if (fb > 0) hipLaunchKernelGGL(spmv_fixup_multi_kernel, dim3((unsigned)fb), dim3(256), 0, stream, d_fix_table, fx, alpha);
    for (int i = 0; i < n; ++i) {
        const SpmvDeviceMatrix& m = *parts[i];
        if (m.n_fix_long > 0)
            hipLaunchKernelGGL(spmv_fixup_long_kernel, dim3((m.n_fix_long + 3) / 4), dim3(256), 0, stream,
                               m.fix_long, m.n_fix_long, m.carry, ys[i], alpha, 0LL, 0LL);
    }
    return hipGetLastError();
}

struct TtsSlice { uint4 v[kSliceSteps]; uint4 m[kSliceSteps]; };
__device__ __forceinline__ void tts_request(TtsSlice& s, const char* words, int slice, int lane) {
    const uint4* pv = (const uint4*)(words + (size_t)slice * (kSliceElems * 8)) + lane;
#pragma unroll
    for (int j = 0; j < kSliceSteps; ++j) s.v[j] = load_words(pv + j * 64);
#pragma unroll
    for (int j = 0; j < kSliceSteps; ++j) s.m[j] = load_words(pv + 256 + j * 64);
}

template <bool HAS_BETA, bool ZERO_FILL = false, int NV = 1, bool XLDS = false, bool GAP = false>
__device__ __forceinline__ void tts_tile_body(const TtsDeviceMatrix& M, const float* __restrict__ x, const float* bias, float* y,
                                              float alpha, float beta, int tile_index, const unsigned tid) {
    extern __shared__ float xs[];
    float* const acc0 = xs;
    float* const staging0 = xs + M.acc_floats * NV;
    const int stage_stride = (NV > 1 || XLDS) ? M.batch_stage_floats : M.staging_floats;
    float* const tails = staging0 + stage_stride * NV;
    float* const xw0 = tails + 64 * NV;
    const int lane = tid & 63, wave = tid >> 6;
    const int wave_u = __builtin_amdgcn_readfirstlane(wave);
    const int n_waves = blockDim.x >> 6;
    constexpr int kE = kSliceSteps * kLaneElems;
    const __amdgpu_buffer_rsrc_t rx = __builtin_amdgcn_make_buffer_rsrc((void*)x, 0, M.cols * NV * 4, 0x00020000);
    const char* const words = (const char*)M.words;
    const int4 tile = load_int4(M.tiles + tile_index);
    const int row0 = tile.x, n_rows = tile.y, block_begin = tile.z, n_blocks = tile.w;

    int4 blk = load_int4(M.blocks + 2 * (size_t)block_begin);
    TtsSlice wA, wB;
    int cbA = 0, cbB = 0;
    if (n_blocks > 0) {
        if (wave < blk.y) { tts_request(wA, words, blk.x + wave, lane); cbA = *(const HISPMV_GLOBAL int*)(M.col_base + blk.x + wave); }
        if (wave + n_waves < blk.y) { tts_request(wB, words, blk.x + wave + n_waves, lane); cbB = *(const HISPMV_GLOBAL int*)(M.col_base + blk.x + wave + n_waves); }
    }
#pragma unroll
    for (int v = 0; v < NV; ++v)
        for (int i = tid; i < n_rows; i += blockDim.x) acc0[v * M.acc_floats + i] = 0.0f;
    if (XLDS) {
        const HISPMV_GLOBAL float* xg = (const HISPMV_GLOBAL float*)x;
        constexpr int kU = kTtsXldsMax / 1024;
        for (int v = 0; v < NV; ++v) {
            float t[kU];
#pragma unroll
            for (int u = 0; u < kU; ++u) { const int i = (int)tid + u * (int)blockDim.x; t[u] = i < M.cols ? xg[(size_t)v * M.cols + i] : 0.0f; }
#pragma unroll
            for (int u = 0; u < kU; ++u) { const int i = (int)tid + u * (int)blockDim.x; if (i < M.xlds_floats) xw0[v * M.xlds_floats + i] = t[u]; }
        }
    }
    if (ZERO_FILL)
        for (int i = tid; i < ((stage_stride * NV) >> 2); i += blockDim.x) ((float4*)staging0)[i] = float4{0.0f, 0.0f, 0.0f, 0.0f};
    __syncthreads();

    auto phase_a = [&](TtsSlice& w, int& cb, int next) {
        const int base0 = __builtin_amdgcn_readfirstlane(cb) << 2;
        const unsigned dummy = (unsigned)stage_stride - 64u;
#pragma unroll 1
        for (int v = 0; v < NV; ++v) {
        const int base = base0 + v * (M.cols << 2);
        float* const staging = staging0 + v * stage_stride;
        float xv[kE];
        if (XLDS) {
            const float* const xw = xw0 + v * M.xlds_floats + (base0 >> 2);
#pragma unroll
            for (int j = 0; j < kSliceSteps; ++j) {
                xv[4 * j + 0] = xw[w.m[j].x >> 16]; xv[4 * j + 1] = xw[w.m[j].y >> 16];
                xv[4 * j + 2] = xw[w.m[j].z >> 16]; xv[4 * j + 3] = xw[w.m[j].w >> 16];
            }
        } else {
#if HISPMV_TTS_EXPERIMENT == 1
#pragma unroll
        for (int j = 0; j < kE; ++j) xv[j] = 1.0f;
        (void)rx; (void)base;
#else
#pragma unroll
        for (int j = 0; j < kSliceSteps; ++j) {
            xv[4 * j + 0] = i2f((int)__builtin_amdgcn_raw_buffer_load_b32(rx, (w.m[j].x >> 16) << 2, base, 0));
            xv[4 * j + 1] = i2f((int)__builtin_amdgcn_raw_buffer_load_b32(rx, (w.m[j].y >> 16) << 2, base, 0));
            xv[4 * j + 2] = i2f((int)__builtin_amdgcn_raw_buffer_load_b32(rx, (w.m[j].z >> 16) << 2, base, 0));
            xv[4 * j + 3] = i2f((int)__builtin_amdgcn_raw_buffer_load_b32(rx, (w.m[j].w >> 16) << 2, base, 0));
        }
#endif
        }
#pragma unroll
        for (int j = 0; j < kSliceSteps; ++j) {
            if (NV > 1 || XLDS) {
                staging[min(w.m[j].x & 0xffffu, dummy)] = i2f((int)w.v[j].x) * xv[4 * j + 0];
                staging[min(w.m[j].y & 0xffffu, dummy)] = i2f((int)w.v[j].y) * xv[4 * j + 1];
                staging[min(w.m[j].z & 0xffffu, dummy)] = i2f((int)w.v[j].z) * xv[4 * j + 2];
                staging[min(w.m[j].w & 0xffffu, dummy)] = i2f((int)w.v[j].w) * xv[4 * j + 3];
            } else {
                staging[w.m[j].x & 0xffffu] = i2f((int)w.v[j].x) * xv[4 * j + 0];
                staging[w.m[j].y & 0xffffu] = i2f((int)w.v[j].y) * xv[4 * j + 1];
                staging[w.m[j].z & 0xffffu] = i2f((int)w.v[j].z) * xv[4 * j + 2];
                staging[w.m[j].w & 0xffffu] = i2f((int)w.v[j].w) * xv[4 * j + 3];
            }
        }
        }
        asm volatile("" ::: "memory");
        if (next >= 0) {
            tts_request(w, words, next, lane);
            cb = *(const HISPMV_GLOBAL int*)(M.col_base + next);
        }
    };
    auto phase_b = [&](int c, int2 ci, unsigned ends) {
#pragma unroll 1
        for (int v = 0; v < NV; ++v) {
        float* const acc = acc0 + v * M.acc_floats;
        int row = __builtin_amdgcn_readfirstlane(ci.x);
        const float4* st4 = (const float4*)(staging0 + v * stage_stride + c * kTtsChunkSlots) + lane;
        float carry_step = 0.0f;
#pragma unroll
// ... 36 lines not shown
#pragma unroll
            for (int k = 0; k < kLaneElems; ++k) a[k] = e[k] ? acc[r[k]] : 0.0f;
#pragma unroll
            for (int k = 0; k < kLaneElems; ++k)
                if (e[k]) acc[r[k]] = a[k] + tj[k];
            row += total;
        }
        if (lane == 0) tails[v * 64 + c] = carry_step;
        }
    };

    for (int b = 0; b < n_blocks; ++b) {
        const int slice_begin = __builtin_amdgcn_readfirstlane(blk.x), n_slices = __builtin_amdgcn_readfirstlane(blk.y);
        const int chunk_begin = __builtin_amdgcn_readfirstlane(blk.z), n_chunks = __builtin_amdgcn_readfirstlane(blk.w);
        int4 nxt = int4{0, 0, 0, 0};
        if (b + 1 < n_blocks) nxt = load_int4(M.blocks + 2 * (size_t)(block_begin + b + 1));
        int2 ciA = int2{0, 0}, ciB = int2{0, 0}, ciT = int2{0, 0};
        unsigned endsA = 0, endsB = 0;
        auto load_ends = [&](int c) -> unsigned {
            if (GAP) return *(const HISPMV_GLOBAL unsigned*)((const unsigned*)M.flags_hi + (size_t)(chunk_begin + c) * 64 + lane);
            return *(const HISPMV_GLOBAL unsigned short*)(M.flags + (size_t)(chunk_begin + c) * 64 + lane);
        };
        if (wave < n_chunks) {
            ciA = load_int2(M.chunk_info + chunk_begin + wave_u);
            endsA = load_ends(wave);
        }
        if (wave + n_waves < n_chunks) {
            ciB = load_int2(M.chunk_info + chunk_begin + wave_u + n_waves);
            endsB = load_ends(wave + n_waves);
        }
        if (wave == 0 && lane < n_chunks) ciT = load_int2(M.chunk_info + chunk_begin + lane);
        const bool more = wave + 2 * n_waves < n_slices;
        if (wave < n_slices) phase_a(wA, cbA, wave < nxt.y ? nxt.x + wave : -1);
        else if (wave < nxt.y) { tts_request(wA, words, nxt.x + wave, lane); cbA = *(const HISPMV_GLOBAL int*)(M.col_base + nxt.x + wave); }
        if (wave + n_waves < n_slices) {
            phase_a(wB, cbB, more ? slice_begin + wave + 2 * n_waves : (wave + n_waves < nxt.y ? nxt.x + wave + n_waves : -1));
            for (int s = wave + 2 * n_waves; s < n_slices; s += n_waves)
                phase_a(wB, cbB, s + n_waves < n_slices ? slice_begin + s + n_waves : (wave + n_waves < nxt.y ? nxt.x + wave + n_waves : -1));
        } else if (wave + n_waves < nxt.y) {
            tts_request(wB, words, nxt.x + wave + n_waves, lane); cbB = *(const HISPMV_GLOBAL int*)(M.col_base + nxt.x + wave + n_waves);
        }
        __syncthreads();
#if HISPMV_TTS_EXPERIMENT != 2
        if (wave < n_chunks) phase_b(wave, ciA, endsA);
        if (wave + n_waves < n_chunks) phase_b(wave + n_waves, ciB, endsB);
        for (int c = wave + 2 * n_waves; c < n_chunks; c += n_waves)
            phase_b(c, load_int2(M.chunk_info + chunk_begin + c), load_ends(c));
#else
        (void)endsA; (void)endsB; (void)ciA; (void)ciB;
#endif
        __syncthreads();
        if (wave == 0 && lane < n_chunks) {
            const int t_chain = GAP ? (ciT.y & 0xffff) : ciT.y;
            const int t_row = GAP ? ciT.x + (ciT.y >> 16) : ciT.x;
            if (t_chain > 0) {
#pragma unroll
                for (int v = 0; v < NV; ++v) {
                    float* const acc = acc0 + v * M.acc_floats;
                    float s = 0.0f;
                    for (int k = lane - t_chain; k < lane; ++k) s += tails[v * 64 + k];
                    acc[t_row] = acc[t_row] + s;
                }
            }
        }
        blk = nxt;
    }
    __syncthreads();
    if (row0 < 0) {
        if ((int)tid < NV) *(HISPMV_GLOBAL float*)(M.carry + (size_t)tid * M.n_carry + (-row0 - 1)) = acc0[tid * M.acc_floats];
        return;
    }
#pragma unroll
    for (int v = 0; v < NV; ++v) {
        const float* const acc = acc0 + v * M.acc_floats;
        float* const yv = y + (size_t)v * M.rows;
        for (int i = tid; i < n_rows; i += blockDim.x) {
            const float t = acc[i];
            if (HAS_BETA) *(HISPMV_GLOBAL float*)(yv + row0 + i) = alpha * t + beta * *(const HISPMV_GLOBAL float*)(bias + row0 + i);
            else *(HISPMV_GLOBAL float*)(yv + row0 + i) = alpha * t;
        }
    }
}

template <bool HAS_BETA, bool ZERO_FILL = false, int NV = 1, bool XLDS = false, bool GAP = false>
__device__ __forceinline__ void tts_tile_body(const TtsDeviceMatrix& M, const float* __restrict__ x, const float* bias, float* y,
                                              float alpha, float beta, int tile_index) {
    tts_tile_body<HAS_BETA, ZERO_FILL, NV, XLDS, GAP>(M, x, bias, y, alpha, beta, tile_index, threadIdx.x);
}
template <bool HAS_BETA, int NV, bool XLDS>
__global__ __launch_bounds__(1024) void spmv_tts_nv_kernel(TtsDeviceMatrix M, const float* __restrict__ x, const float* bias, float* y,
                                                           float alpha, float beta) {
    tts_tile_body<HAS_BETA, false, NV, XLDS>(M, x, bias, y, alpha, beta, (int)blockIdx.x);
}

template <bool HAS_BETA>
__global__ __launch_bounds__(1024) void spmv_tts_kernel(TtsDeviceMatrix M, const float* __restrict__ x, const float* bias, float* y,
                                                        float alpha, float beta) {
    tts_tile_body<HAS_BETA>(M, x, bias, y, alpha, beta, (int)blockIdx.x);
}

template <bool HAS_BETA>
__global__ __launch_bounds__(1024) void spmv_tts_batched_kernel(TtsDeviceMatrix M, const float* __restrict__ x, const float* bias, float* y,
                                                                float alpha, float beta, int nv) {
#pragma unroll 1
    for (int v = 0; v < nv; ++v) {
        tts_tile_body<HAS_BETA>(M, x + (size_t)v * M.cols, bias, y + (size_t)v * M.rows, alpha, beta, (int)blockIdx.x);
        __syncthreads();
        M.carry += M.n_carry;
    }
}

template <bool ZERO_FILL, bool XLDS = false, bool GAP = false>
__global__ __launch_bounds__(1024) void spmv_tts_multi_kernel(const TtsEntry* __restrict__ table, MultiPrefix prefix, float alpha) {
    int k = 0;
#pragma unroll 1
    while (k + 1 < prefix.n && (long long)blockIdx.x >= prefix.begin[k + 1]) ++k;
    int tile = (int)(blockIdx.x - prefix.begin[k]);
    int entry = prefix.first[k];
    const int parts = prefix.tiles[k];
    if (parts > 1) {
        const int per = 8 / parts, res = tile & 7;
        entry += res / per;
        tile = (tile >> 3) * per + (res % per);
    }
    const TtsEntry e = table[entry];
    if (tile >= e.m.n_tiles) return;
    WGT_BEGIN();
    if (e.beta != 0.0f) tts_tile_body<true, ZERO_FILL, 1, XLDS, GAP>(e.m, e.x, e.bias, e.y, alpha, e.beta, tile);
    else tts_tile_body<false, ZERO_FILL, 1, XLDS, GAP>(e.m, e.x, e.y, e.y, alpha, 0.0f, tile);
    WGT_END(3, entry, tile);
}

template <class T>
__device__ __forceinline__ T load_const(const T* p) {
    static_assert(sizeof(T) % 4 == 0, "dword-sized tables");
    typedef const __attribute__((address_space(4))) unsigned* CP;
    union U { T t; unsigned w[sizeof(T) / 4]; __device__ U() {} } u;
    CP src = (CP)(const void*)p;
#pragma unroll
    for (unsigned i = 0; i < sizeof(T) / 4; ++i) u.w[i] = src[i];
    return u.t;
}

template <bool STRAYS>
__global__ __launch_bounds__(1024) void spmv_step_kernel(StepArgs args) {
    extern __shared__ float step_lds[];
    unsigned& s_next = *(unsigned*)(step_lds + args.ticket_word);
    if (threadIdx.x == 0) s_next = __hip_atomic_fetch_add(args.sync, 1u, __ATOMIC_RELAXED, __HIP_MEMORY_SCOPE_AGENT);
    __syncthreads();
#pragma unroll 1
    for (;;) {
        typedef const __attribute__((address_space(4))) StepArgs* KernArgs;
        KernArgs ap = (KernArgs)__builtin_amdgcn_kernarg_segment_ptr();
        asm volatile("" : "+s"(ap));
        const StepArgs a{ap->slice_table, ap->tts_table, ap->items, ap->sync, ap->n_items, ap->alpha, 0, ap->ticket_word};
        unsigned& s_next = *(unsigned*)(step_lds + a.ticket_word);
        const unsigned it = s_next;
        if (it >= a.n_items) break;
        __syncthreads();
        unsigned next = 0;
        if (threadIdx.x == 0) next = __hip_atomic_fetch_add(a.sync, 1u, __ATOMIC_RELAXED, __HIP_MEMORY_SCOPE_AGENT);
        const int2 item = load_const(a.items + __builtin_amdgcn_readfirstlane((int)it));
        const unsigned kind = (unsigned)__builtin_amdgcn_readfirstlane(item.x) & 3u;
        const int entry = (int)((unsigned)__builtin_amdgcn_readfirstlane(item.x) >> 8);
        const long long index = (long long)(unsigned)__builtin_amdgcn_readfirstlane(item.y);
        unsigned tid = threadIdx.x;
        asm volatile("" : "+v"(tid));
        const int wave = __builtin_amdgcn_readfirstlane((int)(tid >> 6));
        WGT_BEGIN();
        if (kind == 2) {
            if (tid == 0) s_next = next;
            const TtsEntry e = load_const(a.tts_table + entry);
            if (e.beta != 0.0f) tts_tile_body<true>(e.m, e.x, e.bias, e.y, a.alpha, e.beta, (int)index, tid);
            else tts_tile_body<false>(e.m, e.x, e.y, e.y, a.alpha, 0.0f, (int)index, tid);
        } else {
            const MultiEntry t = load_const(a.slice_table + entry);
            const LookbackArgs lb{};
            const SubBlock sb = kind == 0 ? SubBlock{wave, 16, 0, (int)(tid & 63)} : SubBlock{wave & 3, 4, (wave >> 2) * (t.lds_floats + 4 * t.ytile_floats), (int)(tid & 63)};
            const long long group = kind == 0 ? index : index + (wave >> 2);
            if (t.beta != 0.0f)
                slices_body<true, true, false, STRAYS>((const char*)t.words, t.hdr, t.groups, t.frags, t.x, t.bias, t.y, t.carry, a.alpha, t.beta,
                                                       t.n_slices, t.group_slices, t.lds_floats, t.ytile_floats, t.cols, t.rows, lb, group, sb);
            else
                slices_body<false, true, false, STRAYS>((const char*)t.words, t.hdr, t.groups, t.frags, t.x, t.y, t.y, t.carry, a.alpha, 0.0f,
                                                        t.n_slices, t.group_slices, t.lds_floats, t.ytile_floats, t.cols, t.rows, lb, group, sb);
            if (tid == 0) s_next = next;
        }
#ifdef HISPMV_WG_TRACE
        WGT_END(kind == 2 ? 3 : kind == 0 ? 1 : 2, entry, index);
#else
        __syncthreads();
#endif
    }
    if (threadIdx.x == 0) {
        unsigned* const sync = ((const __attribute__((address_space(4))) StepArgs*)__builtin_amdgcn_kernarg_segment_ptr())->sync;
        const unsigned done = __hip_atomic_fetch_add(sync + 1, 1u, __ATOMIC_RELAXED, __HIP_MEMORY_SCOPE_AGENT);
        if (done == gridDim.x - 1) {
            __hip_atomic_store(sync + 1, 0u, __ATOMIC_RELAXED, __HIP_MEMORY_SCOPE_AGENT);
            __hip_atomic_store(sync, 0u, __ATOMIC_RELAXED, __HIP_MEMORY_SCOPE_AGENT);
        }
    }
}

template <int NV, bool XLDS>
static hipError_t launch_tts_nv2(const TtsDeviceMatrix& m, const float* x, const float* bias, float* y, float alpha, float beta, hipStream_t stream);

static size_t tts_lds_bytes(const TtsDeviceMatrix& m) { return ((size_t)m.acc_floats + (size_t)m.staging_floats + 64) * sizeof(float); }

hipError_t launch_tts(const TtsDeviceMatrix& m, const float* x, const float* bias, float* y, float alpha, float beta, hipStream_t stream) {
    (void)hipGetLastError();
    if (m.n_tiles <= 0) return hipSuccess;
    static bool raised = false;
    if (!raised) {
        hipError_t e;
        if ((e = hipFuncSetAttribute((const void*)spmv_tts_kernel<true>, hipFuncAttributeMaxDynamicSharedMemorySize, 160 * 1024 - 256)) != hipSuccess) return e;
        if ((e = hipFuncSetAttribute((const void*)spmv_tts_kernel<false>, hipFuncAttributeMaxDynamicSharedMemorySize, 160 * 1024 - 256)) != hipSuccess) return e;
        raised = true;
    }
    const size_t lds = tts_lds_bytes(m);
    if (lds > 160 * 1024 - 256 || m.zero_fill) return hipErrorInvalidValue;
    if (tts_x_in_lds(m, 1)) {
        hipError_t e = launch_tts_nv2<1, true>(m, x, bias, y, alpha, beta, stream);
        if (e != hipSuccess) return e;
    } else
    if (beta != 0.0f) hipLaunchKernelGGL(spmv_tts_kernel<true>, dim3((unsigned)m.n_tiles), dim3(m.threads), lds, stream, m, x, bias, y, alpha, beta);
    else hipLaunchKernelGGL(spmv_tts_kernel<false>, dim3((unsigned)m.n_tiles), dim3(m.threads), lds, stream, m, x, y, y, alpha, beta);
    if (m.n_fix > 0)
        hipLaunchKernelGGL(spmv_fixup_short_kernel, dim3((m.n_fix + 255) / 256), dim3(256), 0, stream, m.fix, m.n_fix, m.carry, y, alpha, 0LL, 0LL);
    return hipGetLastError();
}

static size_t tts_nv_lds_bytes(const TtsDeviceMatrix& m, int nv, bool xlds) {
    return ((size_t)m.acc_floats + (size_t)m.batch_stage_floats + 64 + (xlds ? (size_t)m.xlds_floats : 0)) * nv * sizeof(float);
}
bool tts_x_in_lds(const TtsDeviceMatrix& m, int nv) {
    return !m.zero_fill && m.xlds_floats > 0 && m.batch_stage_floats > 0 && tts_nv_lds_bytes(m, nv, true) <= 160 * 1024 - 256;
}
int tts_batch_width(const TtsDeviceMatrix& m, int64_t vecs) {
    if (vecs < 2 || m.zero_fill || m.batch_stage_floats <= 0) return 1;
    for (int nv = 4; nv >= 2; nv >>= 1)
        if (nv <= vecs && tts_x_in_lds(m, nv)) return nv;
    for (int nv = 4; nv >= 2; nv >>= 1) {
        if (nv > vecs) continue;
        if ((int64_t)m.cols * nv >= (1 << 30) || (int64_t)m.rows * nv >= (1 << 30)) continue;
        if (tts_nv_lds_bytes(m, nv, false) <= 160 * 1024 - 256) return nv;
    }
    return 1;
}

template <bool HAS_BETA, int NV, bool XLDS>
static hipError_t launch_tts_nv(const TtsDeviceMatrix& m, const float* x, const float* bias, float* y, float alpha, float beta, hipStream_t stream) {
    static bool raised = false;
    if (!raised) {
        hipError_t e = hipFuncSetAttribute((const void*)spmv_tts_nv_kernel<HAS_BETA, NV, XLDS>, hipFuncAttributeMaxDynamicSharedMemorySize, 160 * 1024 - 256);
        if (e != hipSuccess) return e;
        raised = true;
    }
    const size_t lds = tts_nv_lds_bytes(m, NV, XLDS);
    hipLaunchKernelGGL((spmv_tts_nv_kernel<HAS_BETA, NV, XLDS>), dim3((unsigned)m.n_tiles), dim3(m.threads), lds, stream, m, x, HAS_BETA ? bias : y, y, alpha, beta);
    return hipGetLastError();
}
template <int NV, bool XLDS>
static hipError_t launch_tts_nv2(const TtsDeviceMatrix& m, const float* x, const float* bias, float* y, float alpha, float beta, hipStream_t stream) {
    return beta != 0.0f ? launch_tts_nv<true, NV, XLDS>(m, x, bias, y, alpha, beta, stream) : launch_tts_nv<false, NV, XLDS>(m, x, bias, y, alpha, beta, stream);
}

hipError_t launch_tts_batched(const TtsDeviceMatrix& m, int nv, const float* x, const float* bias, float* y, float alpha, float beta, hipStream_t stream) {
    (void)hipGetLastError();
    if (nv < 2 || nv > kTtsMaxVectors || m.zero_fill) return hipErrorInvalidValue;
// ... 3 lines not shown
        hipError_t e = nv == 4 ? (xl ? launch_tts_nv2<4, true>(m, x, bias, y, alpha, beta, stream) : launch_tts_nv2<4, false>(m, x, bias, y, alpha, beta, stream))
                               : (xl ? launch_tts_nv2<2, true>(m, x, bias, y, alpha, beta, stream) : launch_tts_nv2<2, false>(m, x, bias, y, alpha, beta, stream));
        if (e != hipSuccess) return e;
        if (m.n_fix > 0)
            hipLaunchKernelGGL(spmv_fixup_short_kernel, dim3((m.n_fix + 255) / 256, nv), dim3(256), 0, stream, m.fix, m.n_fix, m.carry, y, alpha,
                               (long long)m.n_carry, (long long)m.rows);
        return hipGetLastError();
    }
    static bool raised = false;
    if (!raised) {
        hipError_t e;
        if ((e = hipFuncSetAttribute((const void*)spmv_tts_batched_kernel<true>, hipFuncAttributeMaxDynamicSharedMemorySize, 160 * 1024 - 256)) != hipSuccess) return e;
        if ((e = hipFuncSetAttribute((const void*)spmv_tts_batched_kernel<false>, hipFuncAttributeMaxDynamicSharedMemorySize, 160 * 1024 - 256)) != hipSuccess) return e;
        raised = true;
    }
    const size_t lds = tts_lds_bytes(m);
    if (lds > 160 * 1024 - 256) return hipErrorInvalidValue;
    if (beta != 0.0f) hipLaunchKernelGGL(spmv_tts_batched_kernel<true>, dim3((unsigned)m.n_tiles), dim3(m.threads), lds, stream, m, x, bias, y, alpha, beta, nv);
    else hipLaunchKernelGGL(spmv_tts_batched_kernel<false>, dim3((unsigned)m.n_tiles), dim3(m.threads), lds, stream, m, x, y, y, alpha, beta, nv);
    if (m.n_fix > 0)
        hipLaunchKernelGGL(spmv_fixup_short_kernel, dim3((m.n_fix + 255) / 256, nv), dim3(256), 0, stream, m.fix, m.n_fix, m.carry, y, alpha,
                           (long long)m.n_carry, (long long)m.rows);
    return hipGetLastError();
}

hipError_t launch_tts_multi(const TtsEntry* entries, int n, const uint8_t* item_parts, int n_items, const TtsEntry* d_table, float alpha,
                            hipStream_t stream) {
    (void)hipGetLastError();
    if (n <= 0) return hipSuccess;
    if (n > kMultiMax) return hipErrorInvalidValue;
    static bool raised = false;
    if (!raised) {
        hipError_t e;
        if ((e = hipFuncSetAttribute((const void*)spmv_tts_multi_kernel<false>, hipFuncAttributeMaxDynamicSharedMemorySize, 160 * 1024 - 256)) != hipSuccess) return e;
        if ((e = hipFuncSetAttribute((const void*)spmv_tts_multi_kernel<true>, hipFuncAttributeMaxDynamicSharedMemorySize, 160 * 1024 - 256)) != hipSuccess) return e;
        if ((e = hipFuncSetAttribute((const void*)spmv_tts_multi_kernel<false, true>, hipFuncAttributeMaxDynamicSharedMemorySize, 160 * 1024 - 256)) != hipSuccess) return e;
        if ((e = hipFuncSetAttribute((const void*)spmv_tts_multi_kernel<false, false, true>, hipFuncAttributeMaxDynamicSharedMemorySize, 160 * 1024 - 256)) != hipSuccess) return e;
        raised = true;
    }
    if (!item_parts) n_items = n;
    const bool xlds = tts_x_in_lds(entries[0].m, 1);
    MultiPrefix px{};
    px.n = n_items;
    long long g = 0;
    size_t lds = 0;
    int e = 0;
    for (int k = 0; k < n_items; ++k) {
        const int parts = item_parts ? item_parts[k] : 1;
        if ((parts != 1 && parts != 2 && parts != 4) || e + parts > n) return hipErrorInvalidValue;
        if (parts > 1) g = (g + 7) & ~7LL;
        px.begin[k] = g; px.first[k] = (uint8_t)e; px.tiles[k] = (uint8_t)parts;
        long long most = 0;
        for (int q = 0; q < parts; ++q, ++e) {
            most = std::max<long long>(most, entries[e].m.n_tiles);
            lds = std::max(lds, xlds ? tts_nv_lds_bytes(entries[e].m, 1, true) : tts_lds_bytes(entries[e].m));
            if (tts_x_in_lds(entries[e].m, 1) != xlds) return hipErrorInvalidValue;
        }
        if (parts == 1) g += most;
        else { const int per = 8 / parts; g += 8 * ((most + per - 1) / per); }
    }
    if (e != n) return hipErrorInvalidValue;
    px.begin[n_items] = g;
    if (g > 0x7fffffffLL || lds > 160 * 1024 - 256) return hipErrorInvalidValue;
    for (int i = 1; i < n; ++i) if (entries[i].m.zero_fill != entries[0].m.zero_fill || entries[i].m.threads != entries[0].m.threads) return hipErrorInvalidValue;
    if (g > 0 && xlds) hipLaunchKernelGGL((spmv_tts_multi_kernel<false, true>), dim3((unsigned)g), dim3(entries[0].m.threads), lds, stream, d_table, px, alpha);
    else if (g > 0 && entries[0].m.zero_fill == 2) hipLaunchKernelGGL((spmv_tts_multi_kernel<false, false, true>), dim3((unsigned)g), dim3(entries[0].m.threads), lds, stream, d_table, px, alpha);
    else if (g > 0 && entries[0].m.zero_fill) hipLaunchKernelGGL(spmv_tts_multi_kernel<true>, dim3((unsigned)g), dim3(entries[0].m.threads), lds, stream, d_table, px, alpha);
    else if (g > 0) hipLaunchKernelGGL(spmv_tts_multi_kernel<false>, dim3((unsigned)g), dim3(entries[0].m.threads), lds, stream, d_table, px, alpha);
    return hipGetLastError();
}

hipError_t launch_spmv_step(const MultiEntry* d_slice_table, const TtsEntry* d_tts_table, const void* d_items, unsigned n_items,
                            unsigned* d_sync, int workgroups, size_t lds_bytes, bool strays, float alpha, hipStream_t stream) {
    (void)hipGetLastError();
    if (n_items == 0) return hipSuccess;
    if (workgroups <= 0 || lds_bytes > 160 * 1024 - 256) return hipErrorInvalidValue;
    static bool raised = false;
    if (!raised) {
        hipError_t e;
        if ((e = hipFuncSetAttribute((const void*)spmv_step_kernel<false>, hipFuncAttributeMaxDynamicSharedMemorySize, 160 * 1024)) != hipSuccess) return e;
        if ((e = hipFuncSetAttribute((const void*)spmv_step_kernel<true>, hipFuncAttributeMaxDynamicSharedMemorySize, 160 * 1024)) != hipSuccess) return e;
        raised = true;
    }
    const size_t ticket_byte = (lds_bytes + 15) & ~(size_t)15;
    lds_bytes = ticket_byte + 16;
    if (lds_bytes > 160 * 1024) return hipErrorInvalidValue;
    const StepArgs a{d_slice_table, d_tts_table, (const int2*)d_items, d_sync, n_items, alpha, 0, (int)(ticket_byte / 4)};
    if (strays) hipLaunchKernelGGL(spmv_step_kernel<true>, dim3((unsigned)workgroups), dim3(1024), lds_bytes, stream, a);
    else hipLaunchKernelGGL(spmv_step_kernel<false>, dim3((unsigned)workgroups), dim3(1024), lds_bytes, stream, a);
    return hipGetLastError();
}
size_t tts_tile_lds_bytes(const TtsDeviceMatrix& m) { return tts_lds_bytes(m); }

template <int R, bool HAS_BETA, int NV>
__device__ __forceinline__ void gemv_rows_body(const float* __restrict__ W, const float* __restrict__ x,
                                               const float* __restrict__ bias, float* __restrict__ y,
                                               int rows, int cols, float alpha, float beta, int block) {
    __shared__ float part[4][R][NV];
    const int lane = threadIdx.x & 63, wv = threadIdx.x >> 6;
    const int row0 = block * R;
    float acc[R][NV];
#pragma unroll
    for (int r = 0; r < R; ++r)
#pragma unroll
        for (int v = 0; v < NV; ++v) acc[r][v] = 0.0f;

    if ((cols & 3) == 0) {
        const int n4 = cols >> 2;
        const float4* x4 = (const float4*)x;
        for (int c = threadIdx.x; c < n4; c += 256) {
            float4 xv[NV];
#pragma unroll
            for (int v = 0; v < NV; ++v) xv[v] = x4[(size_t)v * n4 + c];
#pragma unroll
            for (int r = 0; r < R; ++r) {
                const int row = min(row0 + r, rows - 1);
                const float4 a = ((const float4*)(W + (size_t)row * cols))[c];
#pragma unroll
                for (int v = 0; v < NV; ++v) acc[r][v] += a.x * xv[v].x + a.y * xv[v].y + a.z * xv[v].z + a.w * xv[v].w;
            }
        }
    } else {
        for (int c = threadIdx.x; c < cols; c += 256) {
            float xv[NV];
#pragma unroll
            for (int v = 0; v < NV; ++v) xv[v] = x[(size_t)v * cols + c];
#pragma unroll
            for (int r = 0; r < R; ++r) {
                const int row = min(row0 + r, rows - 1);
                const float a = W[(size_t)row * cols + c];
#pragma unroll
                for (int v = 0; v < NV; ++v) acc[r][v] += a * xv[v];
            }
        }
    }
#pragma unroll
    for (int r = 0; r < R; ++r)
#pragma unroll
        for (int v = 0; v < NV; ++v) {
            const float s = wave_sum(acc[r][v]);
            if (lane == 0) part[wv][r][v] = s;
        }
    __syncthreads();
    if (threadIdx.x < R * NV) {
        const int r = threadIdx.x / NV, v = threadIdx.x % NV;
        const int row = row0 + r;
        if (row < rows) {
            const float s = (part[0][r][v] + part[1][r][v]) + (part[2][r][v] + part[3][r][v]);
            y[(size_t)v * rows + row] = HAS_BETA ? alpha * s + beta * bias[row] : alpha * s;
        }
    }
}

template <int R, bool HAS_BETA, int NV>
__global__ __launch_bounds__(256) void gemv_rows_kernel(const float* __restrict__ W, const float* __restrict__ x,
                                                        const float* __restrict__ bias, float* __restrict__ y,
                                                        int rows, int cols, float alpha, float beta) {
    gemv_rows_body<R, HAS_BETA, NV>(W, x, bias, y, rows, cols, alpha, beta, (int)blockIdx.x);
}

__global__ __launch_bounds__(256) void gemv_rows_multi_kernel(const GemvEntry* __restrict__ table, MultiPrefix prefix, float alpha) {
    int k = 0;
#pragma unroll 1
    while (k + 1 < prefix.n && (long long)blockIdx.x >= prefix.begin[k + 1]) ++k;
    const GemvEntry e = table[k];
    const int block = (int)((long long)blockIdx.x - prefix.begin[k]);
    if (e.beta != 0.0f) gemv_rows_body<4, true, 1>(e.W, e.x, e.bias, e.y, e.rows, e.cols, alpha, e.beta, block);
    else gemv_rows_body<4, false, 1>(e.W, e.x, e.bias, e.y, e.rows, e.cols, alpha, 0.0f, block);
}

// ... 134 lines not shown
```

hispmv_amd/csrc/hispmv_prep_abi.cpp:

```cpp
#include "hispmv_ctx.h"

using namespace hispmv;

#define g_prep_err (::hispmv::prep_error())

HISPMV_API const char* hispmv_prep_last_error(void) { return g_prep_err.c_str(); }

HISPMV_API int hispmv_host_threads(void) { return host_threads(); }

HISPMV_API int hispmv_prep_from_coo(hispmv_prep** out, const int32_t* r, const int32_t* cl, const float* v,
                                    int64_t nnz, int32_t rows, int32_t cols) {
    if (!out) return HISPMV_EINVAL;
    host_threads();
    *out = nullptr;
    if (rows <= 0 || cols <= 0 || nnz < 0) { g_prep_err = "bad sparse matrix arguments"; return HISPMV_EINVAL; }
    try {
        auto p = std::make_unique<hispmv_prep>();
        p->csr = coo_to_csr(rows, cols, nnz, r, cl, v);
        p->st = build_stream(p->csr);
        *out = p.release();
        return HISPMV_OK;
    } catch (const std::exception& ex) { g_prep_err = ex.what(); return HISPMV_EINVAL; }
}

HISPMV_API int hispmv_prep_from_coo_device(hispmv_prep** out, int device_id, const int32_t* r, const int32_t* cl, const float* v,
                                           int64_t nnz, int32_t rows, int32_t cols, double seconds[5]) {
    if (!out) return HISPMV_EINVAL;
    *out = nullptr;
    if (rows <= 0 || cols <= 0 || nnz < 0 || (nnz > 0 && (!r || !cl || !v))) { g_prep_err = "bad sparse matrix arguments"; return HISPMV_EINVAL; }
    if (hipSetDevice(device_id) != hipSuccess) { g_prep_err = "no such HIP device"; return HISPMV_EDEVICE; }
    try {
        auto p = std::make_unique<hispmv_prep>();
        DevicePrepTimes t;
        std::string err;
        if (!prep_on_device(rows, cols, nnz, r, cl, v, p->csr, p->st, t, err)) {
            g_prep_err = err;
            return err.find("outside") != std::string::npos || err.find("dimension") != std::string::npos ? HISPMV_EINVAL : HISPMV_EDEVICE;
        }
        if (seconds) { seconds[0] = t.upload; seconds[1] = t.csr_device; seconds[2] = t.offsets_host; seconds[3] = t.stream_device; seconds[4] = t.download; }
        *out = p.release();
        return HISPMV_OK;
    } catch (const std::exception& ex) { g_prep_err = ex.what(); return HISPMV_EINVAL; }
}

HISPMV_API int hispmv_prep_from_mtx(hispmv_prep** out, const char* path, int flavor) {
    host_threads();
    if (!out) return HISPMV_EINVAL;
    *out = nullptr;
    if (!path || (flavor != 0 && flavor != 1)) { g_prep_err = "bad arguments"; return HISPMV_EINVAL; }
    try {
        Coo coo = read_mtx(path, (MtxFlavor)flavor);
        auto p = std::make_unique<hispmv_prep>();
        p->csr = coo_to_csr(coo.rows, coo.cols, (int64_t)coo.r.size(), coo.r.data(), coo.c.data(), coo.v.data());
        p->st = build_stream(p->csr);
        *out = p.release();
        return HISPMV_OK;
    } catch (const std::runtime_error& ex) { g_prep_err = ex.what(); return HISPMV_EIO;
    } catch (const std::exception& ex) { g_prep_err = ex.what(); return HISPMV_EINVAL; }
}

HISPMV_API void hispmv_prep_free(hispmv_prep* p) { delete p; }

HISPMV_API int hispmv_prep_choose_format(const hispmv_prep* p, int n_cus, int64_t out[16]) {
    if (!p || !out || n_cus <= 0) return HISPMV_EINVAL;
    try {
        Csr copy = p->csr;
        FormatOptions opt = FormatOptions::from_env();
        opt.decide_only = true;
        const FormatChoice ch = choose_format(std::move(copy), nullptr, n_cus, opt);
        int64_t n_slices = 0, n_elems = 0, n_split = 0, global_elems = 0;
        for (const HostPart& q : ch.parts) {
            if (q.is_tts) { n_slices += (int64_t)q.tts.col_base.size(); n_elems += q.tts.nnz + q.tts.n_fillers; n_split += (int64_t)q.tts.fix.size() / 4; }
            else { n_slices += q.st.n_slices; n_elems += q.st.n_elems; n_split += (int64_t)q.st.fix.size(); global_elems += q.plan.lds_floats > 0 ? q.plan.global_elems : q.st.n_slices * (int64_t)kSliceElems; }
        }
        const HostPart& p0 = ch.parts[0];
        out[0] = ch.format; out[1] = ch.parts.size() > 1 ? (ch.tile_kind ? ch.tile_kind : 1) : 0; out[2] = (int64_t)ch.parts.size();
        out[3] = ch.col_tile_width; out[4] = ch.col_tile_base; out[5] = ch.l2_tiles ? 1 : 0;
        out[6] = ch.format == 1 ? p0.tts.geometry.threads : p0.plan.block_threads;
        out[7] = ch.format == 1 ? p0.tts.geometry.max_slots / kTtsChunk : p0.plan.group_slices;
        out[8] = ch.format == 1 ? 0 : p0.plan.lds_floats;
        out[9] = n_slices; out[10] = n_elems; out[11] = n_split;
        out[12] = (int64_t)(ch.tts_lines_per_gather * 1000.0 + 0.5);
        out[13] = global_elems;
        out[14] = 0; out[15] = 0;
        return HISPMV_OK;
    } catch (const std::exception& ex) { g_prep_err = ex.what(); return HISPMV_EINVAL; }
}

HISPMV_API int hispmv_prep_step_queue(const double* slice_costs, int32_t n_slice, const double* tile_costs, int32_t n_tile, int32_t n_wg, int32_t mode,
                                      int32_t* out_class, int32_t* out_index) {
    if (n_slice < 0 || n_tile < 0 || n_wg <= 0 || mode < 0 || (mode > 4 && mode < 16) || mode > 255 || (n_slice > 0 && !slice_costs) || (n_tile > 0 && !tile_costs) ||
        (n_slice + n_tile > 0 && (!out_class || !out_index))) return HISPMV_EINVAL;
    try {
        const std::vector<double> a(slice_costs, slice_costs + n_slice), b(tile_costs, tile_costs + n_tile);
        const auto order = order_step_queue(a, b, n_wg, mode);
        for (size_t i = 0; i < order.size(); ++i) { out_class[i] = order[i].first; out_index[i] = order[i].second; }
        return HISPMV_OK;
    } catch (const std::exception& ex) { g_prep_err = ex.what(); return HISPMV_EINVAL; }
}

HISPMV_API int hispmv_prep_window_membership(const hispmv_prep* p, int n_cus, uint8_t* inside) {
    if (!p || !inside || n_cus <= 0) return HISPMV_EINVAL;
    try {
        SliceStream copy = build_stream(p->csr);
        const LaunchPlan plan = make_plan(copy, n_cus);
        const std::vector<uint8_t> m = window_membership(p->csr, plan);
        std::copy(m.begin(), m.end(), inside);
        return HISPMV_OK;
    } catch (const std::exception& ex) { g_prep_err = ex.what(); return HISPMV_EINVAL; }
}

HISPMV_API int hispmv_prep_dims(const hispmv_prep* p, int64_t d[8]) {
    if (!p || !d) return HISPMV_EINVAL;
    d[0] = p->st.rows; d[1] = p->st.cols; d[2] = p->st.nnz; d[3] = p->st.n_elems; d[4] = p->st.n_slices;
    d[5] = kSliceElems; d[6] = (int64_t)p->st.fix.size(); d[7] = p->st.bytes();
    return HISPMV_OK;
}
HISPMV_API int hispmv_prep_plan(const hispmv_prep* p, int n_cus, int64_t plan[6]) {
    if (!p || !plan || n_cus <= 0) return HISPMV_EINVAL;
    SliceStream copy = p->st;
    const LaunchPlan g = make_plan(copy, n_cus);
    plan[0] = g.block_threads; plan[1] = g.group_slices; plan[2] = g.lds_floats; plan[3] = g.ytile_floats;
    plan[4] = (int64_t)g.groups.size();
    plan[5] = ((int64_t)g.lds_floats + (int64_t)g.ytile_floats * (g.block_threads / 64)) * 4;
    return HISPMV_OK;
}

HISPMV_API int hispmv_prep_apply_plan(hispmv_prep* p, int n_cus, int64_t counts[2]) {
    if (!p || !counts || n_cus <= 0) return HISPMV_EINVAL;
    p->plan = make_plan(p->st, n_cus);
    counts[0] = (int64_t)p->plan.groups.size(); counts[1] = (int64_t)p->plan.frags.size();
    return HISPMV_OK;
}
HISPMV_API int hispmv_prep_device_stream(hispmv_prep* p, int64_t counts[6]) {
    if (!p || !counts) return HISPMV_EINVAL;
    try {
        p->dstream = pack_device_stream(p->st, p->plan);
        counts[0] = (int64_t)p->dstream.bytes.size(); counts[1] = (int64_t)p->dstream.groups.size() / 4; counts[2] = p->dstream.compact_slices;
        counts[3] = p->dstream.stray_slices; counts[4] = p->dstream.stray_floats; counts[5] = p->plan.lds_floats;
        return HISPMV_OK;
    } catch (const std::exception& ex) { g_prep_err = ex.what(); return HISPMV_EINVAL; }
}
HISPMV_API int hispmv_prep_device_stream_on_device(hispmv_prep* p, int device_id, uint8_t* bytes_out, uint32_t* stray_cols_out) {
    if (!p || !bytes_out) return HISPMV_EINVAL;
    if (p->dstream.groups.empty() || (int64_t)p->st.words.size() != p->st.n_slices * kSliceElems) { g_prep_err = "call hispmv_prep_apply_plan and hispmv_prep_device_stream first"; return HISPMV_ESTATE; }
    if (hipSetDevice(device_id) != hipSuccess) { g_prep_err = "no such HIP device"; return HISPMV_EDEVICE; }
    const int64_t ns = p->st.n_slices;
    const size_t wb = p->st.words.size() * sizeof(uint64_t), gb = p->dstream.groups.size() * sizeof(int32_t), sb = (size_t)ns * kStraySlots * sizeof(uint32_t);
    void *dw = nullptr, *dg = nullptr, *db = nullptr, *ds = nullptr;
    auto done = [&](int rc, const char* what) { if (rc != HISPMV_OK) g_prep_err = what; (void)hipFree(dw); (void)hipFree(dg); (void)hipFree(db); (void)hipFree(ds); return rc; };
    if (hipMalloc(&dw, std::max<size_t>(wb, 8)) != hipSuccess || hipMalloc(&dg, gb) != hipSuccess || hipMalloc(&db, std::max<int64_t>(p->dstream.n_bytes, 8)) != hipSuccess)
        return done(HISPMV_EDEVICE, "hipMalloc failed");
    const bool strays = p->dstream.any_stray && stray_cols_out;
    if (strays && (hipMalloc(&ds, sb) != hipSuccess || hipMemset(ds, 0xff, sb) != hipSuccess)) return done(HISPMV_EDEVICE, "hipMalloc failed");
    if (hipMemcpy(dw, p->st.words.data(), wb, hipMemcpyHostToDevice) != hipSuccess || hipMemcpy(dg, p->dstream.groups.data(), gb, hipMemcpyHostToDevice) != hipSuccess)
        return done(HISPMV_EDEVICE, "hipMemcpy failed");
    if (layout_on_device((const uint64_t*)dw, ns, p->plan.group_slices, (const int32_t*)dg, p->plan.lds_floats, p->plan.block_threads / 64, (uint8_t*)db, (uint32_t*)ds, nullptr) != 0)
        return done(HISPMV_EDEVICE, "layout kernel launch failed");
    if (hipDeviceSynchronize() != hipSuccess) return done(HISPMV_EDEVICE, "layout kernel failed");
    if (hipMemcpy(bytes_out, db, (size_t)p->dstream.n_bytes, hipMemcpyDeviceToHost) != hipSuccess) return done(HISPMV_EDEVICE, "hipMemcpy failed");
    if (strays && hipMemcpy(stray_cols_out, ds, sb, hipMemcpyDeviceToHost) != hipSuccess) return done(HISPMV_EDEVICE, "hipMemcpy failed");
    return done(HISPMV_OK, "");
}
HISPMV_API const void* hispmv_prep_device_array(const hispmv_prep* p, int which) {
    if (!p) return nullptr;
    switch (which) {
        case 0: return p->dstream.bytes.data();
        case 1: return p->dstream.groups.data();
        case 2: return p->dstream.stray_cols.data();
        default: return nullptr;
    }
}
HISPMV_API const int32_t* hispmv_prep_groups(const hispmv_prep* p) { return (const int32_t*)p->plan.groups.data(); }
HISPMV_API const int32_t* hispmv_prep_frags(const hispmv_prep* p) { return (const int32_t*)p->plan.frags.data(); }

HISPMV_API int hispmv_prep_build_tts(hispmv_prep* p, int64_t target_tile_elems, int small_geometry, int64_t counts[8], double* lines_per_gather) {
    if (!p || !counts) return HISPMV_EINVAL;
    try {
        TtsGeometry geo;
// ... 107 lines not shown
```

hispmv_amd/prep.py:

```python
from __future__ import annotations

import ctypes as C
from dataclasses import dataclass

import numpy as np

from ._lib import lib, HISPMV_OK


@dataclass
class Prepared:
    rows: int
    cols: int
    nnz: int
    n_elems: int
    n_slices: int
    slice_elems: int
    stream_bytes: int
    row_ptr: np.ndarray
    col_idx: np.ndarray
    values: np.ndarray
    words: np.ndarray
    hdr: np.ndarray
    fix: np.ndarray
# ... 110 lines not shown
    rc = lib.hispmv_prep_from_coo(C.byref(p), C.c_void_p(r.ctypes.data), C.c_void_p(c.ctypes.data), C.c_void_p(v.ctypes.data), r.size, rows, cols)
    if rc != HISPMV_OK:
        raise ValueError(lib.hispmv_prep_last_error().decode())
    try:
        out = (C.c_int64 * 16)()
        if lib.hispmv_prep_choose_format(p, int(n_cus), out) != HISPMV_OK:
            raise ValueError(lib.hispmv_prep_last_error().decode())
        return dict(zip(FORMAT_FIELDS, (int(x) for x in out)))
    finally:
        lib.hispmv_prep_free(p)


def window_membership(coo_rows, coo_cols, coo_values, rows: int, cols: int, n_cus: int = 256):
    r = np.ascontiguousarray(coo_rows, dtype=np.int32)
    c = np.ascontiguousarray(coo_cols, dtype=np.int32)
    v = np.ascontiguousarray(coo_values, dtype=np.float32)
    p = C.c_void_p()
    if lib.hispmv_prep_from_coo(C.byref(p), C.c_void_p(r.ctypes.data), C.c_void_p(c.ctypes.data), C.c_void_p(v.ctypes.data), r.size, rows, cols) != HISPMV_OK:
        raise ValueError(lib.hispmv_prep_last_error().decode())
    try:
        inside = np.zeros(r.size, dtype=np.uint8)
        if lib.hispmv_prep_window_membership(p, int(n_cus), C.c_void_p(inside.ctypes.data)) != HISPMV_OK:
            raise ValueError(lib.hispmv_prep_last_error().decode())
    finally:
        lib.hispmv_prep_free(p)
    return inside, np.lexsort((np.arange(r.size), c, r))


def device_layout_from_coo(coo_rows, coo_cols, coo_values, rows: int, cols: int, n_cus: int = 256, on_device: int = -1) -> dict:
    r = np.ascontiguousarray(coo_rows, dtype=np.int32)
    c = np.ascontiguousarray(coo_cols, dtype=np.int32)
    v = np.ascontiguousarray(coo_values, dtype=np.float32)
    p = C.c_void_p()
    if lib.hispmv_prep_from_coo(C.byref(p), C.c_void_p(r.ctypes.data), C.c_void_p(c.ctypes.data), C.c_void_p(v.ctypes.data), r.size, rows, cols) != HISPMV_OK:
        raise ValueError(lib.hispmv_prep_last_error().decode())
    try:
        d = (C.c_int64 * 8)()
        lib.hispmv_prep_dims(p, d)
        n_slices, se = int(d[4]), int(d[5])
        words = np.ctypeslib.as_array(lib.hispmv_prep_words(p), shape=(n_slices * se,)).copy()
        pl = (C.c_int64 * 6)()
        lib.hispmv_prep_plan(p, int(n_cus), pl)
        cnt = (C.c_int64 * 2)()
        lib.hispmv_prep_apply_plan(p, int(n_cus), cnt)
        groups = np.ctypeslib.as_array(lib.hispmv_prep_groups(p), shape=(int(cnt[0]) * 4,)).copy().reshape(-1, 4) if cnt[0] else np.zeros((0, 4), np.int32)
        frags = np.ctypeslib.as_array(lib.hispmv_prep_frags(p), shape=(int(cnt[1]) * 4,)).copy().reshape(-1, 4) if cnt[1] else np.zeros((0, 4), np.int32)
        dc = (C.c_int64 * 6)()
        if lib.hispmv_prep_device_stream(p, dc) != HISPMV_OK:
            raise ValueError(lib.hispmv_prep_last_error().decode())

        def arr(which, n, dt):
            ptr = lib.hispmv_prep_device_array(p, which)
            return np.frombuffer((C.c_char * (n * np.dtype(dt).itemsize)).from_address(ptr), dtype=dt).copy() if (n and ptr) else np.zeros(0, dt)
        n_groups = int(dc[1])
        stray_floats = int(dc[4])
        extra = {}
        if on_device >= 0:
            bd = np.zeros(int(dc[0]), np.uint8)
            sd = np.zeros((n_slices, 64) if stray_floats else (0, 64), np.uint32)
            if lib.hispmv_prep_device_stream_on_device(p, int(on_device), C.c_void_p(bd.ctypes.data), C.c_void_p(sd.ctypes.data) if stray_floats else None) != HISPMV_OK:
                raise RuntimeError(lib.hispmv_prep_last_error().decode())
            extra = dict(bytes_device=bd, stray_cols_device=sd)
        return dict(**extra, words=words, n_slices=n_slices, threads=int(pl[0]), group_slices=int(pl[1]), window_floats=int(dc[5]), stray_floats=stray_floats,
                    compact_slices=int(dc[2]), stray_slices=int(dc[3]), groups=groups, frags=frags, bytes=arr(0, int(dc[0]), np.uint8),
                    dgroups=arr(1, n_groups * 4, np.int32).reshape(-1, 4),
                    stray_cols=arr(2, n_slices * 64 if stray_floats else 0, np.uint32).reshape(-1, 64))
    finally:
        lib.hispmv_prep_free(p)


def step_queue(slice_costs, tile_costs, n_wg: int = 256, mode: int = 0):
    a = np.ascontiguousarray(slice_costs, dtype=np.float64)
    b = np.ascontiguousarray(tile_costs, dtype=np.float64)
    n = a.size + b.size
    cls = np.zeros(n, np.int32)
    idx = np.zeros(n, np.int32)
    rc = lib.hispmv_prep_step_queue(C.c_void_p(a.ctypes.data) if a.size else None, a.size, C.c_void_p(b.ctypes.data) if b.size else None, b.size,
                                    int(n_wg), int(mode), C.c_void_p(cls.ctypes.data) if n else None, C.c_void_p(idx.ctypes.data) if n else None)
    if rc != HISPMV_OK:
        raise ValueError("hispmv_prep_step_queue: invalid argument")
    return cls, idx


VALUE_LAYOUT_FIELDS = ("bytes", "map_slots", "chunks", "written", "format", "tile_kind", "parts", "batch_layouts")


def value_layouts_from_coo(coo_rows, coo_cols, coo_values, rows: int, cols: int, n_cus: int = 256) -> dict:
    r = np.ascontiguousarray(coo_rows, dtype=np.int32)
    c = np.ascontiguousarray(coo_cols, dtype=np.int32)
    v = np.ascontiguousarray(coo_values, dtype=np.float32)
    p = C.c_void_p()
    cnt = (C.c_int64 * 8)()
    rc = lib.hispmv_prep_value_layouts(C.byref(p), C.c_void_p(r.ctypes.data), C.c_void_p(c.ctypes.data), C.c_void_p(v.ctypes.data), r.size,
                                       int(rows), int(cols), int(n_cus), cnt)
    if rc != HISPMV_OK:
        raise ValueError(lib.hispmv_prep_last_error().decode())
    try:
        d = dict(zip(VALUE_LAYOUT_FIELDS, (int(x) for x in cnt)))

        def arr(which, n, dt):
            ptr = lib.hispmv_prep_value_array(p, which)
            return np.frombuffer((C.c_char * (n * np.dtype(dt).itemsize)).from_address(ptr), dtype=dt).copy() if (n and ptr) else np.zeros(0, dt)
        d.update(real=arr(0, d["bytes"], np.uint8), index=arr(1, d["bytes"], np.uint8), map=arr(2, d["map_slots"], np.int32),
                 chunks=arr(3, 2 * d["chunks"], np.int64).reshape(-1, 2))
        return d
    finally:
        lib.hispmv_prep_free(p)
```

include/hispmv.h:

```cpp
#ifndef HISPMV_H
#define HISPMV_H

#include <stdint.h>

#ifdef __cplusplus
extern "C" {
#endif

#define HISPMV_OK          0
#define HISPMV_FULL       -1
#define HISPMV_EINVAL     -2
#define HISPMV_EDEVICE    -3
#define HISPMV_ESTATE     -4
#define HISPMV_ENOTDENSE  -5
#define HISPMV_EIO        -6
#define HISPMV_ENOMEM     -7

typedef struct hispmv_ctx hispmv_ctx;

int hispmv_create(hispmv_ctx** out, const char* xclbin_path, int device_id,
                  int num_ch_A, int num_ch_B, int num_ch_C, int urams_per_pe, int fp_acc_latency,
                  int dense_overlay, int pre_accumulator, int row_dist_net);

void hispmv_destroy(hispmv_ctx* ctx);
// ... 14 lines not shown
int hispmv_create_dense_handle(hispmv_ctx* ctx, const float* flattened_dense_values, int32_t rows, int32_t cols);

int hispmv_load_matrices(hispmv_ctx* ctx);

int hispmv_select_matrix(hispmv_ctx* ctx, uint32_t matrix_idx);

int hispmv_run_kernel(hispmv_ctx* ctx, const float* x, const float* bias, float* y, float alpha, float beta);

int hispmv_linear(hispmv_ctx* ctx, int matrix_idx, const float* x, int64_t x_len, const float* bias, float* y_out);

int hispmv_spmv_device(hispmv_ctx* ctx, int matrix_idx, const float* d_x, const float* d_bias, float* d_y,
                       float alpha, float beta, void* stream);
int hispmv_synchronize(hispmv_ctx* ctx);

float hispmv_last_kernel_ms(hispmv_ctx* ctx);

int hispmv_batch_graph_stats(hispmv_ctx* ctx, int64_t out[2]);
int hispmv_batch_call_info(hispmv_ctx* ctx, int64_t out[4]);

int hispmv_spmv_device_batch(hispmv_ctx* ctx, int32_t n, const int32_t* idx, const float* const* d_x,
                             const float* const* d_bias, float* const* d_y, float alpha, float beta, void* stream);

int hispmv_set_value_updates(hispmv_ctx* ctx, int enable);
int hispmv_update_values(hispmv_ctx* ctx, int matrix_idx, const float* values, int64_t n);
int hispmv_update_values_device(hispmv_ctx* ctx, int matrix_idx, const float* d_values, int64_t n, void* stream);
int hispmv_value_update_info(const hispmv_ctx* ctx, int matrix_idx, int64_t out[4]);

float hispmv_time_device(hispmv_ctx* ctx, int matrix_idx, const float* d_x, const float* d_bias, float* d_y,
                         float alpha, float beta, int reps);

int hispmv_boundary_pack(hispmv_ctx* ctx, const float* const* d_last, const float* d_mask, float* d_send, int32_t n, void* stream);
int hispmv_boundary_apply(hispmv_ctx* ctx, float* const* d_first, const float* d_recv, const float* d_weights, int32_t n, int32_t world,
                          void* stream);

typedef struct hispmv_matrix_info {
    int32_t rows, cols;
    int64_t nnz;
    int32_t is_dense;
    int32_t loaded;
    int64_t n_slices;
    int64_t n_elems;
    int64_t n_split_rows;
    int64_t device_bytes;
    double prep_seconds;
    int32_t block_threads;
    int32_t group_slices;
    int32_t lds_bytes;
    int32_t col_tiles;
    int32_t carry_lookback;
    int32_t col_tile_width;
    int32_t col_tile_base;
    int32_t compact_slices;
    int32_t format;
    float tts_lines_per_gather;
    int32_t tile_kind;
    int32_t batch_group_slices;
} hispmv_matrix_info;
int hispmv_get_matrix_info(const hispmv_ctx* ctx, int matrix_idx, hispmv_matrix_info* out);
int hispmv_num_matrices(const hispmv_ctx* ctx);

typedef struct hispmv_prep hispmv_prep;
int hispmv_prep_from_coo(hispmv_prep** out, const int32_t* coo_rows, const int32_t* coo_cols,
                         const float* coo_values, int64_t nnz, int32_t rows, int32_t cols);
int hispmv_prep_from_mtx(hispmv_prep** out, const char* mtx_path, int flavor);
int hispmv_prep_from_coo_device(hispmv_prep** out, int device_id, const int32_t* coo_rows, const int32_t* coo_cols,
                                const float* coo_values, int64_t nnz, int32_t rows, int32_t cols, double seconds[5]);
void hispmv_prep_free(hispmv_prep* p);
const char* hispmv_prep_last_error(void);
int hispmv_prep_dims(const hispmv_prep* p, int64_t dims[8]);
const int64_t* hispmv_prep_csr_row_ptr(const hispmv_prep* p);
const int32_t* hispmv_prep_csr_col(const hispmv_prep* p);
const float* hispmv_prep_csr_val(const hispmv_prep* p);
const uint64_t* hispmv_prep_words(const hispmv_prep* p);
const int32_t* hispmv_prep_slice_hdr(const hispmv_prep* p);
const int32_t* hispmv_prep_fix(const hispmv_prep* p);

int hispmv_prep_plan(const hispmv_prep* p, int n_cus, int64_t plan[6]);

int hispmv_prep_choose_format(const hispmv_prep* p, int n_cus, int64_t out[16]);

int hispmv_prep_step_queue(const double* slice_costs, int32_t n_slice, const double* tile_costs, int32_t n_tile, int32_t n_wg, int32_t mode,
                           int32_t* out_class, int32_t* out_index);

int hispmv_prep_window_membership(const hispmv_prep* p, int n_cus, uint8_t* inside);

int hispmv_prep_apply_plan(hispmv_prep* p, int n_cus, int64_t counts[2]);
const int32_t* hispmv_prep_groups(const hispmv_prep* p);
int hispmv_prep_device_stream(hispmv_prep* p, int64_t counts[6]);
const void* hispmv_prep_device_array(const hispmv_prep* p, int which);
int hispmv_prep_device_stream_on_device(hispmv_prep* p, int device_id, uint8_t* bytes_out, uint32_t* stray_cols_out);
const int32_t* hispmv_prep_frags(const hispmv_prep* p);

int hispmv_prep_value_layouts(hispmv_prep** out, const int32_t* coo_rows, const int32_t* coo_cols, const float* coo_values, int64_t nnz,
                              int32_t rows, int32_t cols, int n_cus, int64_t counts[8]);
const void* hispmv_prep_value_array(const hispmv_prep* p, int which);

int64_t hispmv_free_failures(void);

int hispmv_prep_build_tts(hispmv_prep* p, int64_t target_tile_elems, int small_geometry, int64_t counts[8], double* lines_per_gather);
const void* hispmv_prep_tts_array(const hispmv_prep* p, int which);
int hispmv_prep_tts_pieces(const hispmv_prep* p, int64_t counts[2]);

int hispmv_host_threads(void);

const char* hispmv_version(void);

#ifdef __cplusplus
}
#endif
#endif
```

Before: 1317.

## Pack self-contained step-queue item descriptors and prefetch next item into LDS

Each queue entry of the persistent step kernel now carries a 128-byte descriptor holding the group or tile/block metadata it needs, built on the host from kept host copies of the group, tile and block tables. The kernel can then park the next item's descriptor in LDS ahead of time (HISPMV_STEP_AHEAD) instead of chasing dependent global loads for group and tile metadata at the start of each item. This removes a serialized latency chain per work item and also drops the device-to-host readback of tile tables during plan build. In exchange the items array is much larger, more LDS is reserved per workgroup, and extra host memory is kept per matrix.

```diff
diff --git a/hispmv_amd/_lib.py b/hispmv_amd/_lib.py
--- a/hispmv_amd/_lib.py
+++ b/hispmv_amd/_lib.py
@@ -81,6 +81,7 @@
     "hispmv_prep_plan": (C.c_int, [_p, C.c_int, _i64p]),
     "hispmv_prep_choose_format": (C.c_int, [_p, C.c_int, _i64p]),
     "hispmv_prep_step_queue": (C.c_int, [_p, C.c_int32, _p, C.c_int32, C.c_int32, C.c_int32, _p, _p]),
+    "hispmv_prep_step_items": (C.c_int, [_p, C.c_int32, _p, _p, _p, _p, C.c_int32, _p, _p, _p, _p, C.c_int32, _p, _p]),
     "hispmv_prep_window_membership": (C.c_int, [_p, C.c_int, C.c_void_p]),
     "hispmv_prep_apply_plan": (C.c_int, [_p, C.c_int, _i64p]),
     "hispmv_prep_groups": (_i32p, [_p]),
diff --git a/hispmv_amd/csrc/hispmv_abi.cpp b/hispmv_amd/csrc/hispmv_abi.cpp
--- a/hispmv_amd/csrc/hispmv_abi.cpp
+++ b/hispmv_amd/csrc/hispmv_abi.cpp
@@ -543,6 +543,9 @@
             TtsDeviceMatrix& d = p.tdev;
             d.words = dw; d.col_base = dcb; d.flags = dfl; d.flags_hi = dfh; d.chunk_info = (const int2*)dci; d.tiles = (const int4*)dt; d.blocks = (const int4*)db;
             d.n_tiles = (int32_t)ts.tiles.size(); d.rows = m.rows; d.cols = m.cols;
+            static_assert(sizeof(TtsTile) == 16 && sizeof(TtsBlock) == 32, "tile / block tables: 4 / 8 words per entry");
+            p.h_tiles.assign((const int32_t*)ts.tiles.data(), (const int32_t*)ts.tiles.data() + ts.tiles.size() * 4);
+            p.h_blocks.assign((const int32_t*)ts.blocks.data(), (const int32_t*)ts.blocks.data() + ts.blocks.size() * 8);
             if (!ts.fix.empty()) {
                 const int32_t* dfix = nullptr;
                 if ((rc = upload(c, m, ts.fix.data(), ts.fix.size(), &dfix)) != HISPMV_OK) return rc;
@@ -569,6 +572,7 @@
                 const int32_t* dg = nullptr; const Frag* dfr = nullptr;
                 const int64_t ns = p.st.n_slices;
                 if ((rc = upload(c, m, p.dstream.groups.data(), p.dstream.groups.size(), &dg)) != HISPMV_OK) return rc;
+                p.h_groups = p.dstream.groups;
                 if ((rc = upload(c, m, p.plan.frags.data(), p.plan.frags.size(), &dfr)) != HISPMV_OK) return rc;
                 const bool lay_out = p.dstream.bytes.empty() && p.dstream.n_bytes > 0;
                 uint64_t* d_host_words = nullptr;
@@ -659,6 +663,7 @@
                     SpmvDeviceMatrix b = d;
                     const int32_t* bg = nullptr; const Frag* bf = nullptr; const uint8_t* bw = nullptr; const SliceHdr* bh = nullptr;
                     if ((rc = upload(c, m, p.batch_dstream.groups.data(), p.batch_dstream.groups.size(), &bg)) != HISPMV_OK) return rc;
+                    p.h_batch_groups = p.batch_dstream.groups;
                     if ((rc = upload(c, m, p.batch_plan.frags.data(), p.batch_plan.frags.size(), &bf)) != HISPMV_OK) return rc;
                     std::vector<SliceHdr> bhh = hh;
                     for (int64_t sl = 0; sl < ns; ++sl) bhh[(size_t)sl].x_span = (!p.batch_plan.slice_spills.empty() && p.batch_plan.slice_spills[(size_t)sl]) ? 1 : 0;
diff --git a/hispmv_amd/csrc/hispmv_batch.cpp b/hispmv_amd/csrc/hispmv_batch.cpp
--- a/hispmv_amd/csrc/hispmv_batch.cpp
+++ b/hispmv_amd/csrc/hispmv_batch.cpp
@@ -16,6 +16,38 @@
         for (auto& l : p.launches) { dev_free(l.d_table); dev_free(l.d_table2); dev_free(l.d_items); dev_free(l.d_sync); }
     }
     c->batch_plans.clear();
+}
+
+bool pack_step_items(const uint32_t* items, size_t n, const StepSliceTable* slice_tables, size_t n_slice_tables,
+                     const StepTileTable* tile_tables, size_t n_tile_tables, StepItem* out) {
+    for (size_t i = 0; i < n; ++i) {
+        const uint32_t kind = items[2 * i] & 0xffu, entry = items[2 * i] >> 8, index = items[2 * i + 1];
+        StepItem it{};
+        it.kind_entry = items[2 * i]; it.index = index;
+        if (kind == 0 || kind == 1) {
+            if (entry >= n_slice_tables) return false;
+            const StepSliceTable& t = slice_tables[entry];
+            if (!t.groups || t.group_slices <= 0 || (int64_t)index >= t.n_groups || (int64_t)index * t.group_slices >= t.n_slices) return false;
+            for (int64_t q = 0; q < (kind == 0 ? 1 : 4); ++q) {
+                const int64_t g = (int64_t)index + q;
+                if (g < t.n_groups && g * t.group_slices < t.n_slices) std::memcpy(&it.d[q], t.groups + 4 * g, sizeof(int4));
+            }
+        } else if (kind == 2) {
+            if (entry >= n_tile_tables) return false;
+            const StepTileTable& t = tile_tables[entry];
+            if (!t.tiles || (int64_t)index >= t.n_tiles) return false;
+            const int32_t* tile = t.tiles + 4 * (int64_t)index;
+            if (tile[3] <= 0 || tile[2] < 0 || !t.blocks || (int64_t)tile[2] + tile[3] > t.n_blocks) return false;
+            const int32_t* blk = t.blocks + 8 * (int64_t)tile[2];
+            if (blk[1] <= 0) return false;
+            std::memcpy(&it.d[0], tile, sizeof(int4));
+            std::memcpy(&it.d[1], blk, 2 * sizeof(int4));
+        } else {
+            return false;
+        }
+        out[i] = it;
+    }
+    return true;
 }
 
 }
@@ -210,6 +242,22 @@
             std::vector<QItem> q[2];
             std::vector<MultiEntry> slice_table;
             std::vector<TtsEntry> tts_table;
+            std::vector<StepSliceTable> slice_host;
+            std::vector<StepTileTable> tile_host;
+            auto host_groups_of = [&](const SpmvDeviceMatrix* d) -> const std::vector<int32_t>* {
+                for (int i = 0; i < n; ++i)
+                    for (const Matrix::Part& p : c->mats[idx[i]]->parts) {
+                        if (d == &p.dev) return &p.h_groups;
+                        if (d == &p.batch_dev) return &p.h_batch_groups;
+                    }
+                return nullptr;
+            };
+            auto host_part_of = [&](const TtsDeviceMatrix& t) -> const Matrix::Part* {
+                for (int i = 0; i < n; ++i)
+                    for (const Matrix::Part& p : c->mats[idx[i]]->parts)
+                        if (c->mats[idx[i]]->format == 1 && p.tdev.words == t.words && p.tdev.tiles == t.tiles) return &p;
+                return nullptr;
+            };
             for (const auto& l : plan.launches) {
                 if (l.kind == 0) {
                     for (size_t e = 0; e < l.multi.size(); ++e) {
@@ -217,6 +265,8 @@
                         const uint32_t entry = (uint32_t)slice_table.size();
                         slice_table.push_back(l.multi[e]);
                         const int64_t ng = d.n_slices > 0 ? d.n_groups : 0;
+                        const std::vector<int32_t>* hg = host_groups_of(&d);
+                        slice_host.push_back(StepSliceTable{hg ? hg->data() : nullptr, hg ? (int64_t)(hg->size() / 4) : 0, d.n_slices, d.group_slices});
                         const bool window = d.lds_floats > 0;
                         const double per_slice = window ? 0.27 : 0.68;
                         if (d.block_threads == 1024) {
@@ -237,12 +287,14 @@
                     for (const TtsEntry& te : l.tts) {
                         const uint32_t entry = (uint32_t)tts_table.size();
                         tts_table.push_back(te);
-                        std::vector<int4> tiles((size_t)te.m.n_tiles);
-                        HIP_TRY(c, hipMemcpy(tiles.data(), te.m.tiles, tiles.size() * sizeof(int4), hipMemcpyDeviceToHost));
-                        int n_blocks = 0;
-                        for (const int4& t : tiles) n_blocks = std::max(n_blocks, t.z + t.w);
-                        std::vector<int4> blocks((size_t)n_blocks * 2);
-                        if (n_blocks > 0) HIP_TRY(c, hipMemcpy(blocks.data(), te.m.blocks, blocks.size() * sizeof(int4), hipMemcpyDeviceToHost));
+                        const Matrix::Part* hp = host_part_of(te.m);
+                        if (!hp || hp->h_tiles.size() != (size_t)te.m.n_tiles * 4) return fail(c, HISPMV_ESTATE, "internal: host copy of a tile table missing");
+                        const int4* const tiles = (const int4*)hp->h_tiles.data();
+                        const int4* const blocks = (const int4*)hp->h_blocks.data();
+                        const int64_t n_blocks = (int64_t)(hp->h_blocks.size() / 8);
+                        for (int t = 0; t < te.m.n_tiles; ++t)
+                            if (tiles[t].z < 0 || tiles[t].w < 0 || (int64_t)tiles[t].z + tiles[t].w > n_blocks) return fail(c, HISPMV_ESTATE, "internal: tile table out of range");
+                        tile_host.push_back(StepTileTable{hp->h_tiles.data(), te.m.n_tiles, hp->h_blocks.data(), n_blocks});
                         double lines = 23.0;
                         for (int i = 0; i < n; ++i) { const Matrix& m = *c->mats[idx[i]]; if (!m.dense && m.format == 1 && m.parts[0].tdev.words == te.m.words && m.tts_lines_per_gather > 0) lines = m.tts_lines_per_gather; }
                         static const double tile_scale = std::getenv("HISPMV_STEP_TILE_SCALE") ? std::atof(std::getenv("HISPMV_STEP_TILE_SCALE")) : 1.0;
@@ -255,7 +307,8 @@
                     }
                 }
             }
-            if (slice_table.size() < (1u << 20) && tts_table.size() < (1u << 20) && !q[0].empty()) {
+            if (slice_table.size() < (1u << 20) && tts_table.size() < (1u << 20) && !q[0].empty() &&
+                (uint64_t)q[0].size() + q[1].size() + (uint64_t)std::max(1, c->n_cus) <= 0xffffffffull) {
                 const int W = std::max(1, c->n_cus);
                 std::vector<double> cost[2];
                 for (int k = 0; k < 2; ++k) for (const QItem& it : q[k]) cost[k].push_back(it.cost);
@@ -264,35 +317,38 @@
                 std::vector<uint32_t> packed;
                 packed.reserve(order.size() * 2);
                 for (const QItem& it : order) { packed.push_back(it.a); packed.push_back(it.b); }
-                hispmv_ctx::BatchLaunch L;
-                L.kind = 6;
-                L.n_items = (unsigned)order.size();
-                L.step_workgroups = (int)std::min<size_t>((size_t)W, order.size());
-                L.step_lds = lds;
-                L.step_strays = strays;
-                for (const auto& l : plan.launches) L.weight += l.weight;
-                std::vector<hispmv_ctx::BatchLaunch> keep;
-                for (auto& l : plan.launches) {
-                    if (l.kind == 0 || l.kind == 3) { dev_free(l.d_table); dev_free(l.d_table2); }
-                    else keep.push_back(std::move(l));
-                }
-                plan.launches.clear();
-                plan.launches.push_back(std::move(L));
-                for (auto& l : keep) plan.launches.push_back(std::move(l));
-                hispmv_ctx::BatchLaunch& S = plan.launches.front();
-                if (!slice_table.empty()) {
-                    HIP_TRY(c, hipMalloc(&S.d_table, slice_table.size() * sizeof(MultiEntry)));
-                    HIP_TRY(c, hipMemcpy(S.d_table, slice_table.data(), slice_table.size() * sizeof(MultiEntry), hipMemcpyHostToDevice));
-                }
-                if (!tts_table.empty()) {
-                    HIP_TRY(c, hipMalloc(&S.d_table2, tts_table.size() * sizeof(TtsEntry)));
-                    HIP_TRY(c, hipMemcpy(S.d_table2, tts_table.data(), tts_table.size() * sizeof(TtsEntry), hipMemcpyHostToDevice));
-                }
-                HIP_TRY(c, hipMalloc(&S.d_items, packed.size() * sizeof(uint32_t)));
-                HIP_TRY(c, hipMemcpy(S.d_items, packed.data(), packed.size() * sizeof(uint32_t), hipMemcpyHostToDevice));
-                HIP_TRY(c, hipMalloc((void**)&S.d_sync, 2 * sizeof(unsigned)));
-                HIP_TRY(c, hipMemset(S.d_sync, 0, 2 * sizeof(unsigned)));
-                step_taken = true;
+                std::vector<StepItem> descs(order.size());
+                step_taken = pack_step_items(packed.data(), order.size(), slice_host.data(), slice_host.size(), tile_host.data(), tile_host.size(), descs.data());
+                if (step_taken) {
+                    hispmv_ctx::BatchLaunch L;
+                    L.kind = 6;
+                    L.n_items = (unsigned)order.size();
+                    L.step_workgroups = (int)std::min<size_t>((size_t)W, order.size());
+                    L.step_lds = lds;
+                    L.step_strays = strays;
+                    for (const auto& l : plan.launches) L.weight += l.weight;
+                    std::vector<hispmv_ctx::BatchLaunch> keep;
+                    for (auto& l : plan.launches) {
+                        if (l.kind == 0 || l.kind == 3) { dev_free(l.d_table); dev_free(l.d_table2); }
+                        else keep.push_back(std::move(l));
+                    }
+                    plan.launches.clear();
+                    plan.launches.push_back(std::move(L));
+                    for (auto& l : keep) plan.launches.push_back(std::move(l));
+                    hispmv_ctx::BatchLaunch& S = plan.launches.front();
+                    if (!slice_table.empty()) {
+                        HIP_TRY(c, hipMalloc(&S.d_table, slice_table.size() * sizeof(MultiEntry)));
+                        HIP_TRY(c, hipMemcpy(S.d_table, slice_table.data(), slice_table.size() * sizeof(MultiEntry), hipMemcpyHostToDevice));
+                    }
+                    if (!tts_table.empty()) {
+                        HIP_TRY(c, hipMalloc(&S.d_table2, tts_table.size() * sizeof(TtsEntry)));
+                        HIP_TRY(c, hipMemcpy(S.d_table2, tts_table.data(), tts_table.size() * sizeof(TtsEntry), hipMemcpyHostToDevice));
+                    }
+                    HIP_TRY(c, hipMalloc(&S.d_items, descs.size() * sizeof(StepItem)));
+                    HIP_TRY(c, hipMemcpy(S.d_items, descs.data(), descs.size() * sizeof(StepItem), hipMemcpyHostToDevice));
+                    HIP_TRY(c, hipMalloc((void**)&S.d_sync, 2 * sizeof(unsigned)));
+                    HIP_TRY(c, hipMemset(S.d_sync, 0, 2 * sizeof(unsigned)));
+                }
             }
         }
     }
diff --git a/hispmv_amd/csrc/hispmv_ctx.h b/hispmv_amd/csrc/hispmv_ctx.h
--- a/hispmv_amd/csrc/hispmv_ctx.h
+++ b/hispmv_amd/csrc/hispmv_ctx.h
@@ -40,6 +40,8 @@
         hispmv::SpmvDeviceMatrix dev;
         hispmv::SpmvDeviceMatrix batch_dev;
         bool has_batch_dev = false;
+        std::vector<int32_t> h_groups, h_batch_groups;
+        std::vector<int32_t> h_tiles, h_blocks;
     };
     std::vector<Part> parts;
     std::vector<float> dense_host;
@@ -182,6 +184,11 @@
 }
 
 int check_device_error(hispmv_ctx* c);
+
+struct StepSliceTable { const int32_t* groups; int64_t n_groups; int64_t n_slices; int32_t group_slices; };
+struct StepTileTable { const int32_t* tiles; int64_t n_tiles; const int32_t* blocks; int64_t n_blocks; };
+bool pack_step_items(const uint32_t* items, size_t n, const StepSliceTable* slice_tables, size_t n_slice_tables,
+                     const StepTileTable* tile_tables, size_t n_tile_tables, StepItem* out);
 void free_batch_plans(hispmv_ctx* c);
 int spmv_batch_locked(hispmv_ctx* c, int32_t n, const int32_t* idx, const float* const* d_x, const float* const* d_bias,
                       float* const* d_y, float alpha, float beta, hipStream_t s);
diff --git a/hispmv_amd/csrc/hispmv_kernels.h b/hispmv_amd/csrc/hispmv_kernels.h
--- a/hispmv_amd/csrc/hispmv_kernels.h
+++ b/hispmv_amd/csrc/hispmv_kernels.h
@@ -126,7 +126,17 @@
 hipError_t launch_tts_multi(const TtsEntry* entries, int n, const uint8_t* item_parts, int n_items, const TtsEntry* d_table, float alpha,
                             hipStream_t stream);
 
-struct StepArgs { const MultiEntry* slice_table; const TtsEntry* tts_table; const int2* items; unsigned* sync; unsigned n_items; float alpha; int pad, ticket_word; };
+struct alignas(128) StepItem {
+    uint32_t kind_entry;
+    uint32_t index;
+    uint32_t pad[2];
+    int4 d[4];
+    uint32_t pad2[12];
+};
+static_assert(sizeof(StepItem) == 128 && alignof(StepItem) == 128, "StepItem: one 128-byte line");
+constexpr int kStepItemBytes = (int)sizeof(StepItem);
+constexpr int kStepParkBytes = 2 * kStepItemBytes + 16;
+struct StepArgs { const MultiEntry* slice_table; const TtsEntry* tts_table; const StepItem* items; unsigned* sync; unsigned n_items; float alpha; int pad, park_word; };
 hipError_t launch_spmv_step(const MultiEntry* d_slice_table, const TtsEntry* d_tts_table, const void* d_items, unsigned n_items,
                             unsigned* d_sync, int workgroups, size_t lds_bytes, bool strays, float alpha, hipStream_t stream);
 size_t tts_tile_lds_bytes(const TtsDeviceMatrix& m);
diff --git a/hispmv_amd/csrc/hispmv_kernels.hip b/hispmv_amd/csrc/hispmv_kernels.hip
--- a/hispmv_amd/csrc/hispmv_kernels.hip
+++ b/hispmv_amd/csrc/hispmv_kernels.hip
@@ -140,6 +140,11 @@
 __device__ __forceinline__ int4 load_int4(const int4* p) {
     typedef int i4v __attribute__((ext_vector_type(4)));
     const i4v v = *(const HISPMV_GLOBAL i4v*)p;
+    return int4{v.x, v.y, v.z, v.w};
+}
+__device__ __forceinline__ int4 load_int4_lds(const int4* p) {
+    typedef int i4v __attribute__((ext_vector_type(4)));
+    const i4v v = *(const __attribute__((address_space(3))) i4v*)p;
     return int4{v.x, v.y, v.z, v.w};
 }
 __device__ __forceinline__ float4 load_float4(const float4* p) {
@@ -547,6 +552,19 @@
                                                        lds_floats, ytile_floats, cols, rows, lb, group, int4{0, 0, 0, 0}, sb);
     }
 }
+template <bool HAS_BETA, bool STRAYS>
+__device__ __forceinline__ void slices_body(
+    const char* __restrict__ stream, const int4* __restrict__ hdr, const int4* __restrict__ groups,
+    const int4* __restrict__ frags, const float* __restrict__ x, const float* bias, float* y,
+    float* __restrict__ carry, float alpha, float beta, long long n_slices, int group_slices,
+    int lds_floats, int ytile_floats, int cols, int rows, const LookbackArgs& lb, long long group, const SubBlock sb, const int4 g) {
+    if (__builtin_amdgcn_readfirstlane(g.w) != 0)
+        slices_group<HAS_BETA, true, false, true, STRAYS>(stream, hdr, groups, frags, x, bias, y, carry, alpha, beta, n_slices, group_slices,
+                                                          lds_floats, ytile_floats, cols, rows, lb, group, g, sb);
+    else
+        slices_group<HAS_BETA, true, false, false>(stream, hdr, groups, frags, x, bias, y, carry, alpha, beta, n_slices, group_slices,
+                                                   lds_floats, ytile_floats, cols, rows, lb, group, g, sb);
+}
 template <bool HAS_BETA, bool USE_LDS, bool LOOKBACK, bool STRAYS = false>
 __device__ __forceinline__ void slices_body(
     const char* __restrict__ stream, const int4* __restrict__ hdr, const int4* __restrict__ groups,
@@ -1122,9 +1140,9 @@
     for (int j = 0; j < kSliceSteps; ++j) s.m[j] = load_words(pv + 256 + j * 64);
 }
 
-template <bool HAS_BETA, bool ZERO_FILL = false, int NV = 1, bool XLDS = false, bool GAP = false>
+template <bool HAS_BETA, bool ZERO_FILL = false, int NV = 1, bool XLDS = false, bool GAP = false, int DESC = 0>
 __device__ __forceinline__ void tts_tile_body(const TtsDeviceMatrix& M, const float* __restrict__ x, const float* bias, float* y,
-                                              float alpha, float beta, int tile_index, const unsigned tid) {
+                                              float alpha, float beta, int tile_index, const unsigned tid, const int4* desc = nullptr) {
     extern __shared__ float xs[];
     float* const acc0 = xs;
     float* const staging0 = xs + M.acc_floats * NV;
@@ -1137,10 +1155,10 @@
     constexpr int kE = kSliceSteps * kLaneElems;
     const __amdgpu_buffer_rsrc_t rx = __builtin_amdgcn_make_buffer_rsrc((void*)x, 0, M.cols * NV * 4, 0x00020000);
     const char* const words = (const char*)M.words;
-    const int4 tile = load_int4(M.tiles + tile_index);
+    const int4 tile = DESC == 2 ? load_int4_lds(desc) : DESC == 1 ? load_int4(desc) : load_int4(M.tiles + tile_index);
     const int row0 = tile.x, n_rows = tile.y, block_begin = tile.z, n_blocks = tile.w;
 
-    int4 blk = load_int4(M.blocks + 2 * (size_t)block_begin);
+    int4 blk = DESC == 2 ? load_int4_lds(desc + 1) : DESC == 1 ? load_int4(desc + 1) : load_int4(M.blocks + 2 * (size_t)block_begin);
     TtsSlice wA, wB;
     int cbA = 0, cbB = 0;
     if (n_blocks > 0) {
@@ -1343,6 +1361,11 @@
     }
 }
 
+template <bool HAS_BETA, int DESC>
+__device__ __forceinline__ void tts_tile_body(const TtsDeviceMatrix& M, const float* __restrict__ x, const float* bias, float* y,
+                                              float alpha, float beta, const int4* desc, const unsigned tid) {
+    tts_tile_body<HAS_BETA, false, 1, false, false, DESC>(M, x, bias, y, alpha, beta, 0, tid, desc);
+}
 template <bool HAS_BETA, bool ZERO_FILL = false, int NV = 1, bool XLDS = false, bool GAP = false>
 __device__ __forceinline__ void tts_tile_body(const TtsDeviceMatrix& M, const float* __restrict__ x, const float* bias, float* y,
                                               float alpha, float beta, int tile_index) {
@@ -1403,49 +1426,101 @@
     return u.t;
 }
 
+#ifndef HISPMV_STEP_AHEAD
+#define HISPMV_STEP_AHEAD 1
+#endif
+constexpr int kStepSlotFloats = kStepItemBytes / 4;
+constexpr int kStepTicketFloat = 2 * kStepSlotFloats;
+
+__device__ __forceinline__ void step_request_item(const StepItem* items, unsigned ticket, unsigned n_items, float* slot, unsigned tid) {
+    if (ticket < n_items && tid < (unsigned)(kStepItemBytes / 16)) {
+        const char* const src = (const char*)(items + ticket) + tid * 16;
+        const unsigned dst = (unsigned)(size_t)(__attribute__((address_space(3))) float*)slot;
+        unsigned keep;
+        asm volatile("s_mov_b32 %0, m0\n\ts_mov_b32 m0, %2\n\ts_nop 0\n\tglobal_load_lds_dwordx4 %1, off\n\ts_mov_b32 m0, %0"
+                     : "=&s"(keep) : "v"(src), "s"(dst) : "memory");
+    }
+}
+
 template <bool STRAYS>
 __global__ __launch_bounds__(1024) void spmv_step_kernel(StepArgs args) {
     extern __shared__ float step_lds[];
-    unsigned& s_next = *(unsigned*)(step_lds + args.ticket_word);
-    if (threadIdx.x == 0) s_next = __hip_atomic_fetch_add(args.sync, 1u, __ATOMIC_RELAXED, __HIP_MEMORY_SCOPE_AGENT);
+#if HISPMV_STEP_AHEAD
+    if (threadIdx.x < 64) {
+        unsigned t0 = 0;
+        if (threadIdx.x == 0) {
+            t0 = __hip_atomic_fetch_add(args.sync, 1u, __ATOMIC_RELAXED, __HIP_MEMORY_SCOPE_AGENT);
+            *(uint2*)(step_lds + args.park_word + kStepTicketFloat) = uint2{t0, 0u};
+        }
+        step_request_item(args.items, (unsigned)__builtin_amdgcn_readfirstlane((int)t0), args.n_items, step_lds + args.park_word, threadIdx.x);
+        asm volatile("s_waitcnt vmcnt(0)" ::: "memory");
+    }
+#else
+    if (threadIdx.x == 0) *(unsigned*)(step_lds + args.park_word + kStepTicketFloat) = __hip_atomic_fetch_add(args.sync, 1u, __ATOMIC_RELAXED, __HIP_MEMORY_SCOPE_AGENT);
+#endif
     __syncthreads();
 #pragma unroll 1
     for (;;) {
         typedef const __attribute__((address_space(4))) StepArgs* KernArgs;
         KernArgs ap = (KernArgs)__builtin_amdgcn_kernarg_segment_ptr();
         asm volatile("" : "+s"(ap));
-        const StepArgs a{ap->slice_table, ap->tts_table, ap->items, ap->sync, ap->n_items, ap->alpha, 0, ap->ticket_word};
-        unsigned& s_next = *(unsigned*)(step_lds + a.ticket_word);
+        const StepArgs a{ap->slice_table, ap->tts_table, ap->items, ap->sync, ap->n_items, ap->alpha, 0, ap->park_word};
+        float* const park = step_lds + a.park_word;
+        unsigned tid = threadIdx.x;
+        asm volatile("" : "+v"(tid));
+        const int wave = __builtin_amdgcn_readfirstlane((int)(tid >> 6));
+#if HISPMV_STEP_AHEAD
+        const uint2 tk = *(const uint2*)(park + kStepTicketFloat);
+        if (tk.x >= a.n_items) break;
+        __syncthreads();
+        const int slot = __builtin_amdgcn_readfirstlane((int)tk.y);
+        unsigned next = 0;
+        if (tid == 0) {
+            next = __hip_atomic_fetch_add(a.sync, 1u, __ATOMIC_RELAXED, __HIP_MEMORY_SCOPE_AGENT);
+            *(uint2*)(park + kStepTicketFloat) = uint2{next, (unsigned)(slot ^ 1)};
+        }
+        step_request_item(a.items, (unsigned)__builtin_amdgcn_readfirstlane((int)next), a.n_items, park + (slot ^ 1) * kStepSlotFloats, tid);
+        const int4* const desc = (const int4*)(park + slot * kStepSlotFloats);
+        const uint2 head = *(const uint2*)desc;
+        const unsigned kind = (unsigned)__builtin_amdgcn_readfirstlane((int)head.x) & 3u;
+#else
+        unsigned& s_next = *(unsigned*)(park + kStepTicketFloat);
         const unsigned it = s_next;
         if (it >= a.n_items) break;
         __syncthreads();
         unsigned next = 0;
-        if (threadIdx.x == 0) next = __hip_atomic_fetch_add(a.sync, 1u, __ATOMIC_RELAXED, __HIP_MEMORY_SCOPE_AGENT);
-        const int2 item = load_const(a.items + __builtin_amdgcn_readfirstlane((int)it));
-        const unsigned kind = (unsigned)__builtin_amdgcn_readfirstlane(item.x) & 3u;
-        const int entry = (int)((unsigned)__builtin_amdgcn_readfirstlane(item.x) >> 8);
-        const long long index = (long long)(unsigned)__builtin_amdgcn_readfirstlane(item.y);
-        unsigned tid = threadIdx.x;
-        asm volatile("" : "+v"(tid));
-        const int wave = __builtin_amdgcn_readfirstlane((int)(tid >> 6));
+        if (tid == 0) next = __hip_atomic_fetch_add(a.sync, 1u, __ATOMIC_RELAXED, __HIP_MEMORY_SCOPE_AGENT);
+        const int4* const desc = (const int4*)(a.items + __builtin_amdgcn_readfirstlane((int)it));
+        const uint2 head = load_const((const uint2*)desc);
+        const unsigned kind = (unsigned)__builtin_amdgcn_readfirstlane((int)head.x) & 3u;
+        if (kind == 2 && tid == 0) s_next = next;
+#endif
+        const int entry = (int)((unsigned)__builtin_amdgcn_readfirstlane((int)head.x) >> 8);
+        const long long index = (long long)(unsigned)__builtin_amdgcn_readfirstlane((int)head.y);
         WGT_BEGIN();
         if (kind == 2) {
-            if (tid == 0) s_next = next;
             const TtsEntry e = load_const(a.tts_table + entry);
-            if (e.beta != 0.0f) tts_tile_body<true>(e.m, e.x, e.bias, e.y, a.alpha, e.beta, (int)index, tid);
-            else tts_tile_body<false>(e.m, e.x, e.y, e.y, a.alpha, 0.0f, (int)index, tid);
+            if (e.beta != 0.0f) tts_tile_body<true, HISPMV_STEP_AHEAD ? 2 : 1>(e.m, e.x, e.bias, e.y, a.alpha, e.beta, desc + 1, tid);
+            else tts_tile_body<false, HISPMV_STEP_AHEAD ? 2 : 1>(e.m, e.x, e.y, e.y, a.alpha, 0.0f, desc + 1, tid);
         } else {
+#if HISPMV_STEP_AHEAD
+            const int4 g = load_int4_lds(desc + 1 + (kind == 1 ? wave >> 2 : 0));
+#else
+            const int4 g = load_int4(desc + 1 + (kind == 1 ? wave >> 2 : 0));
+#endif
             const MultiEntry t = load_const(a.slice_table + entry);
             const LookbackArgs lb{};
             const SubBlock sb = kind == 0 ? SubBlock{wave, 16, 0, (int)(tid & 63)} : SubBlock{wave & 3, 4, (wave >> 2) * (t.lds_floats + 4 * t.ytile_floats), (int)(tid & 63)};
             const long long group = kind == 0 ? index : index + (wave >> 2);
             if (t.beta != 0.0f)
-                slices_body<true, true, false, STRAYS>((const char*)t.words, t.hdr, t.groups, t.frags, t.x, t.bias, t.y, t.carry, a.alpha, t.beta,
-                                                       t.n_slices, t.group_slices, t.lds_floats, t.ytile_floats, t.cols, t.rows, lb, group, sb);
+                slices_body<true, STRAYS>((const char*)t.words, t.hdr, t.groups, t.frags, t.x, t.bias, t.y, t.carry, a.alpha, t.beta,
+                                          t.n_slices, t.group_slices, t.lds_floats, t.ytile_floats, t.cols, t.rows, lb, group, sb, g);
             else
-                slices_body<false, true, false, STRAYS>((const char*)t.words, t.hdr, t.groups, t.frags, t.x, t.y, t.y, t.carry, a.alpha, 0.0f,
-                                                        t.n_slices, t.group_slices, t.lds_floats, t.ytile_floats, t.cols, t.rows, lb, group, sb);
+                slices_body<false, STRAYS>((const char*)t.words, t.hdr, t.groups, t.frags, t.x, t.y, t.y, t.carry, a.alpha, 0.0f,
+                                           t.n_slices, t.group_slices, t.lds_floats, t.ytile_floats, t.cols, t.rows, lb, group, sb, g);
+#if !HISPMV_STEP_AHEAD
             if (tid == 0) s_next = next;
+#endif
         }
 #ifdef HISPMV_WG_TRACE
         WGT_END(kind == 2 ? 3 : kind == 0 ? 1 : 2, entry, index);
@@ -1615,10 +1690,11 @@
         if ((e = hipFuncSetAttribute((const void*)spmv_step_kernel<true>, hipFuncAttributeMaxDynamicSharedMemorySize, 160 * 1024)) != hipSuccess) return e;
         raised = true;
     }
-    const size_t ticket_byte = (lds_bytes + 15) & ~(size_t)15;
-    lds_bytes = ticket_byte + 16;
+    const size_t park_byte = (lds_bytes + 15) & ~(size_t)15;
+    lds_bytes = park_byte + (size_t)kStepParkBytes;
     if (lds_bytes > 160 * 1024) return hipErrorInvalidValue;
-    const StepArgs a{d_slice_table, d_tts_table, (const int2*)d_items, d_sync, n_items, alpha, 0, (int)(ticket_byte / 4)};
+    if ((unsigned long long)n_items + (unsigned long long)workgroups > 0xffffffffull) return hipErrorInvalidValue;
+    const StepArgs a{d_slice_table, d_tts_table, (const StepItem*)d_items, d_sync, n_items, alpha, 0, (int)(park_byte / 4)};
     if (strays) hipLaunchKernelGGL(spmv_step_kernel<true>, dim3((unsigned)workgroups), dim3(1024), lds_bytes, stream, a);
     else hipLaunchKernelGGL(spmv_step_kernel<false>, dim3((unsigned)workgroups), dim3(1024), lds_bytes, stream, a);
     return hipGetLastError();
diff --git a/hispmv_amd/csrc/hispmv_prep_abi.cpp b/hispmv_amd/csrc/hispmv_prep_abi.cpp
--- a/hispmv_amd/csrc/hispmv_prep_abi.cpp
+++ b/hispmv_amd/csrc/hispmv_prep_abi.cpp
@@ -95,6 +95,29 @@
         const std::vector<double> a(slice_costs, slice_costs + n_slice), b(tile_costs, tile_costs + n_tile);
         const auto order = order_step_queue(a, b, n_wg, mode);
         for (size_t i = 0; i < order.size(); ++i) { out_class[i] = order[i].first; out_index[i] = order[i].second; }
+        return HISPMV_OK;
+    } catch (const std::exception& ex) { g_prep_err = ex.what(); return HISPMV_EINVAL; }
+}
+
+HISPMV_API int hispmv_prep_step_items(const uint32_t* items, int32_t n, const int32_t* const* group_tables, const int64_t* group_counts,
+                                      const int64_t* slice_counts, const int32_t* group_slices, int32_t n_slice_entries,
+                                      const int32_t* const* tile_tables, const int64_t* tile_counts, const int32_t* const* block_tables,
+                                      const int64_t* block_counts, int32_t n_tile_entries, void* out, int32_t out_layout[4]) {
+    if (out_layout) { out_layout[0] = (int32_t)sizeof(StepItem); out_layout[1] = (int32_t)alignof(StepItem); out_layout[2] = (int32_t)offsetof(StepItem, d); out_layout[3] = kStepParkBytes; }
+    if (n < 0 || n_slice_entries < 0 || n_tile_entries < 0 || (n > 0 && (!items || !out)) ||
+        (n_slice_entries > 0 && (!group_tables || !group_counts || !slice_counts || !group_slices)) ||
+        (n_tile_entries > 0 && (!tile_tables || !tile_counts || !block_tables || !block_counts))) return HISPMV_EINVAL;
+    try {
+        std::vector<StepSliceTable> st((size_t)n_slice_entries);
+        for (int e = 0; e < n_slice_entries; ++e) st[(size_t)e] = StepSliceTable{group_tables[e], group_counts[e], slice_counts[e], group_slices[e]};
+        std::vector<StepTileTable> tt((size_t)n_tile_entries);
+        for (int e = 0; e < n_tile_entries; ++e) tt[(size_t)e] = StepTileTable{tile_tables[e], tile_counts[e], block_tables[e], block_counts[e]};
+        std::vector<StepItem> packed((size_t)n);
+        if (!pack_step_items(items, (size_t)n, st.data(), st.size(), tt.data(), tt.size(), packed.data())) {
+            g_prep_err = "hispmv_prep_step_items: an item outside its table, or one without a first slice";
+            return HISPMV_EINVAL;
+        }
+        if (n > 0) std::memcpy(out, packed.data(), packed.size() * sizeof(StepItem));
         return HISPMV_OK;
     } catch (const std::exception& ex) { g_prep_err = ex.what(); return HISPMV_EINVAL; }
 }
diff --git a/hispmv_amd/prep.py b/hispmv_amd/prep.py
--- a/hispmv_amd/prep.py
+++ b/hispmv_amd/prep.py
@@ -216,6 +216,30 @@
     return cls, idx
 
 
+def step_items(entries, slice_tables=(), tile_tables=()):
+    e = np.ascontiguousarray(entries, dtype=np.uint32).reshape(-1, 2)
+    groups = [np.ascontiguousarray(t[0], dtype=np.int32).reshape(-1, 4) for t in slice_tables]
+    tiles = [np.ascontiguousarray(t[0], dtype=np.int32).reshape(-1, 4) for t in tile_tables]
+    blocks = [np.ascontiguousarray(t[1], dtype=np.int32).reshape(-1, 8) for t in tile_tables]
+
+    def ptrs(arrs):
+        return (C.c_void_p * max(1, len(arrs)))(*[a.ctypes.data for a in arrs])
+
+    def counts(vals, ct):
+        return (ct * max(1, len(vals)))(*[int(v) for v in vals])
+    layout = (C.c_int32 * 4)()
+    lib.hispmv_prep_step_items(None, 0, None, None, None, None, 0, None, None, None, None, 0, None, layout)
+    out = np.zeros((e.shape[0], layout[0] // 4), np.uint32)
+    rc = lib.hispmv_prep_step_items(C.c_void_p(e.ctypes.data) if e.size else None, e.shape[0],
+                                    ptrs(groups), counts([g.shape[0] for g in groups], C.c_int64), counts([t[1] for t in slice_tables], C.c_int64),
+                                    counts([t[2] for t in slice_tables], C.c_int32), len(groups),
+                                    ptrs(tiles), counts([t.shape[0] for t in tiles], C.c_int64), ptrs(blocks), counts([b.shape[0] for b in blocks], C.c_int64),
+                                    len(tiles), C.c_void_p(out.ctypes.data) if e.size else None, layout)
+    if rc != HISPMV_OK:
+        raise ValueError(lib.hispmv_prep_last_error().decode())
+    return out, dict(item_bytes=int(layout[0]), alignment=int(layout[1]), table_offset=int(layout[2]), park_bytes=int(layout[3]))
+
+
 VALUE_LAYOUT_FIELDS = ("bytes", "map_slots", "chunks", "written", "format", "tile_kind", "parts", "batch_layouts")
 
 
diff --git a/include/hispmv.h b/include/hispmv.h
--- a/include/hispmv.h
+++ b/include/hispmv.h
@@ -120,6 +120,11 @@
 int hispmv_prep_step_queue(const double* slice_costs, int32_t n_slice, const double* tile_costs, int32_t n_tile, int32_t n_wg, int32_t mode,
                            int32_t* out_class, int32_t* out_index);
 
+int hispmv_prep_step_items(const uint32_t* items, int32_t n, const int32_t* const* group_tables, const int64_t* group_counts,
+                           const int64_t* slice_counts, const int32_t* group_slices, int32_t n_slice_entries,
+                           const int32_t* const* tile_tables, const int64_t* tile_counts, const int32_t* const* block_tables,
+                           const int64_t* block_counts, int32_t n_tile_entries, void* out, int32_t out_layout[4]);
+
 int hispmv_prep_window_membership(const hispmv_prep* p, int n_cus, uint8_t* inside);
 
 int hispmv_prep_apply_plan(hispmv_prep* p, int n_cus, int64_t counts[2]);
```

Result: faster. 1332, median of 6 (+1.2%).
